# skhu101/TDNN-F_NAS

Measured on AMD Instinct MI355X. Metric: LF-MMI training frames/sec per node (SWBD 7q TDNN-F), higher is better.
Workload: dtype f32

## Files before the change

### include/tdnnf_hip.h

```cpp
#ifndef TDNNF_HIP_H_
#define TDNNF_HIP_H_

#include <stddef.h>
#include <stdint.h>

#ifdef __cplusplus
extern "C" {
#endif

#define TDNNF_OK 0
#define TDNNF_EINVAL 1
#define TDNNF_EHIP 2

#define TDNNF_MAX_OFFSETS 16

typedef struct {
  float *data;
  int rows, cols, stride;
} tdnnf_mat;

typedef void *tdnnf_stream;
typedef struct tdnnf_ng tdnnf_ng;

const char *tdnnf_last_error(void);
// ... 67 lines not shown
int tdnnf_batchnorm_compute_derived(const double *stats_dev, int D, float epsilon, float target_rms,
                                    float *scale_dev, float *offset_dev, tdnnf_stream stream);
int tdnnf_batchnorm_test_propagate(const tdnnf_mat *in, const float *scale_dev, const float *offset_dev,
                                   tdnnf_mat *out, tdnnf_stream stream);
int tdnnf_batchnorm_test_backprop(const tdnnf_mat *out_deriv, const float *scale_dev, tdnnf_mat *in_deriv,
                                  tdnnf_stream stream);


int tdnnf_softmax_flops_propagate(const tdnnf_mat *in, const float *gumbel_u_dev, float temp_proportion,
                                  tdnnf_mat *out, tdnnf_stream stream);
int tdnnf_softmax_flops_backprop(const tdnnf_mat *out_value, tdnnf_mat *out_deriv, float scale,
                                 const float *flops_dev, int dim, float temp_proportion,
                                 tdnnf_mat *in_deriv, tdnnf_stream stream);
int tdnnf_onehot_propagate(const float *sample_u_dev, tdnnf_mat *out, tdnnf_stream stream);
int tdnnf_onehot_backprop(const tdnnf_mat *out_deriv, float lr, float *output_acc_dev, void *workspace_dev,
                          size_t workspace_bytes, tdnnf_stream stream);
int tdnnf_copyn_propagate(const tdnnf_mat *in, float scale, tdnnf_mat *out, tdnnf_stream stream);
int tdnnf_copyn_backprop(const tdnnf_mat *out_deriv, float scale, tdnnf_mat *in_deriv, tdnnf_stream stream);
int tdnnf_constant_function_propagate(const float *output_dev, tdnnf_mat *out, tdnnf_stream stream);
int tdnnf_constant_function_backprop(const tdnnf_mat *out_deriv, float lr, float *output_acc_dev,
                                     void *workspace_dev, size_t workspace_bytes, tdnnf_stream stream);
int tdnnf_flops_constraint_backprop(const float *flops_dev, float scale, int rows_in, int cols_in,
                                    tdnnf_mat *in_deriv, tdnnf_stream stream);

int tdnnf_elementwise_product_propagate(const tdnnf_mat *in, int output_dim, tdnnf_mat *out, tdnnf_stream);
int tdnnf_elementwise_product_backprop(const tdnnf_mat *in_value, const tdnnf_mat *out_deriv, int output_dim,
                                       tdnnf_mat *in_deriv, tdnnf_stream);
int tdnnf_relu_propagate(const tdnnf_mat *in, tdnnf_mat *out, tdnnf_stream);
int tdnnf_relu_backprop(const tdnnf_mat *out_value, const tdnnf_mat *out_deriv, tdnnf_mat *in_deriv, tdnnf_stream);
int tdnnf_relu_repair(const double *stats_dev, int dim, float self_repair_scale, float lower, float upper,
                      tdnnf_mat *in_deriv, tdnnf_stream);
int tdnnf_relu_store_stats(const tdnnf_mat *out_value, double *stats_dev, void *workspace_dev,
                           size_t workspace_bytes, tdnnf_stream);
int tdnnf_affine_propagate(const tdnnf_mat *in, const float *W_dev, int ldw, const float *bias_dev, int Do,
                           tdnnf_mat *out, tdnnf_stream);
int tdnnf_affine_backprop(const tdnnf_mat *out_deriv, const float *W_dev, int ldw, int Di, tdnnf_mat *in_deriv,
                          tdnnf_stream);
int tdnnf_affine_update_simple(const tdnnf_mat *in_value, const tdnnf_mat *out_deriv, float lr, float *W_acc_dev,
                               int ldw, float *bias_acc_dev, void *workspace_dev, size_t workspace_bytes,
                               tdnnf_stream);
size_t tdnnf_affine_update_natural_gradient_workspace_bytes(int Do, int Di, int num_rows, int has_bias);
int tdnnf_affine_update_natural_gradient(const tdnnf_mat *in_value, const tdnnf_mat *out_deriv,
                                         tdnnf_ng *preconditioner_in, tdnnf_ng *preconditioner_out,
                                         float learning_rate, float *W_acc_dev, int ldw, float *bias_acc_dev,
                                         void *workspace_dev, size_t workspace_bytes, tdnnf_stream);
int tdnnf_log_softmax_propagate(const tdnnf_mat *in, tdnnf_mat *out, tdnnf_stream);
int tdnnf_log_softmax_backprop(const tdnnf_mat *out_value, const tdnnf_mat *out_deriv, tdnnf_mat *in_deriv,
                               tdnnf_stream);
int tdnnf_sum_scaled(const tdnnf_mat *a, float sa, const tdnnf_mat *b, float sb, tdnnf_mat *out, tdnnf_stream);
int tdnnf_add_scaled(const tdnnf_mat *a, float s, tdnnf_mat *out, tdnnf_stream);
int tdnnf_general_dropout(const tdnnf_mat *in, const float *mask_dev, int num_seq, tdnnf_mat *out, tdnnf_stream);
int tdnnf_general_dropout_mask(const float *uniform_dev, long long n, float proportion, int continuous, float *mask_dev, tdnnf_stream);

typedef struct tdnnf_den_graph tdnnf_den_graph;
typedef struct tdnnf_supervision tdnnf_supervision;

int tdnnf_den_graph_create(int num_states, int num_arcs, int num_pdfs, const int *arc_src, const int *arc_dst,
                           const int *arc_pdf, const float *arc_prob, const float *initial_probs, int start_state,
                           tdnnf_den_graph **out);
void tdnnf_den_graph_destroy(tdnnf_den_graph *);
int tdnnf_supervision_create(int num_sequences, int frames_per_sequence, const int *seq_state_begin,
                             const int *seq_arc_begin, const int *state_time, const float *final_logprob,
                             const int *arc_src, const int *arc_dst, const int *arc_pdf, const float *arc_logprob,
                             float weight, tdnnf_supervision **out);
void tdnnf_supervision_destroy(tdnnf_supervision *);

int tdnnf_chain_set_denominator_mode(int mode);
int tdnnf_chain_den_mw_status(int *fallbacks, int *disabled, int reset);
size_t tdnnf_chain_workspace_bytes(const tdnnf_den_graph *, int num_sequences, int frames_per_sequence);
int tdnnf_chain_objf_and_deriv(const tdnnf_den_graph *, const tdnnf_supervision *, const tdnnf_mat *nnet_output,
                               const tdnnf_mat *xent_output , float leaky_hmm_coefficient,
                               float l2_regularize, float xent_regularize, double *results_dev,
                               tdnnf_mat *nnet_output_deriv, tdnnf_mat *xent_deriv, void *workspace_dev,
                               size_t workspace_bytes, tdnnf_stream);

int tdnnf_ng_create(int rank, int update_period, float num_samples_history, float alpha, tdnnf_ng **out);
void tdnnf_ng_destroy(tdnnf_ng *);
int tdnnf_ng_freeze(tdnnf_ng *, int freeze);
int tdnnf_ng_precondition(tdnnf_ng *, tdnnf_mat *X, float *scale_host, tdnnf_stream);
size_t tdnnf_ng_stats_pass_workspace_bytes(int rank, int Di, int num_taps, int N);
int tdnnf_ng_stats_pass(const tdnnf_tdnn_indexes *ix, const tdnnf_mat *X, int Di, const float *eff_dev, const float *WT_dev,
                        const float *W_dev, int ldw, const float *bias_dev, tdnnf_mat *H, double *sumsq_dev, int sumsq_cap, int form,
                        void *workspace_dev, size_t workspace_bytes, tdnnf_stream);
const float *tdnnf_ng_scale_dev(const tdnnf_ng *);

size_t tdnnf_constrain_orthonormal_workspace_bytes(int rows, int cols);
int tdnnf_constrain_orthonormal(float scale, float *M_dev, int rows, int cols, int ld, void *workspace_dev,
                                size_t workspace_bytes, tdnnf_stream);
int tdnnf_axpy(const float *x_dev, float a, float *y_dev, size_t n, tdnnf_stream);
int tdnnf_dot(const float *x_dev, const float *y_dev, size_t n, double *result_host, tdnnf_stream);
size_t tdnnf_max_change_workspace_bytes(int num_comp);
int tdnnf_update_with_max_change(float *params_dev, float *delta_dev, int num_comp, const long long *comp_begin_host,
                                 const float *max_change_host, float max_param_change, float max_change_scale,
                                 float scale, int zero_delta, void *workspace_dev, size_t workspace_bytes,
                                 float *info_dev, tdnnf_stream);

int tdnnf_splice_input(const tdnnf_mat *feats, const tdnnf_mat *ivectors, int num_seq, int num_splice,
                       tdnnf_mat *out, tdnnf_stream);
int tdnnf_reorder_rows(const tdnnf_mat *in, int num_seq, int rho, int to_rho, tdnnf_mat *out, tdnnf_stream);

#define TDNNF_NET_MAX_LAYERS 32
typedef struct {
  int feat_dim, ivector_dim, num_pdfs;
  int hidden_dim, prefinal_small_dim;
  int num_layers;
  int bottleneck_dim[TDNNF_NET_MAX_LAYERS];
  int time_stride[TDNNF_NET_MAX_LAYERS];
  float bypass_scale;
  int frames_per_chunk, num_sequences;
  int frame_subsampling;
  float leaky_hmm, xent_regularize, chain_l2_regularize;
  float l2_hidden, l2_output;
  float max_change_hidden, max_change_output, max_param_change;
  float relu_self_repair_scale;
  float batchnorm_stats_scale;
  int darts_num_offsets;
  int darts_flags;
  float darts_temp_proportion;
  int use_natural_gradient;
  int bn_num_choices;
  int bn_choice_dims[8];
  int bn_mode;
  float bn_flops_scale;
  float bn_temp_proportion;
  int cv_update;
  int gemm_precision;
  int use_layer_offsets;
  int offset_left[TDNNF_NET_MAX_LAYERS];
  int offset_right[TDNNF_NET_MAX_LAYERS];
  int use_dropout;
} tdnnf_net_config;
typedef struct tdnnf_net tdnnf_net;

typedef struct tdnnf_egs_reader tdnnf_egs_reader;
typedef struct tdnnf_egs_writer tdnnf_egs_writer;
typedef struct tdnnf_eg tdnnf_eg;
int tdnnf_egs_reader_open(const char *path, tdnnf_egs_reader **out);
void tdnnf_egs_reader_close(tdnnf_egs_reader *);
int tdnnf_egs_reader_next(tdnnf_egs_reader *, tdnnf_eg **out);
void tdnnf_eg_destroy(tdnnf_eg *);
const char *tdnnf_eg_key(const tdnnf_eg *);
int tdnnf_eg_input_info(const tdnnf_eg *, const char *name, int *rows, int *cols, int *first_t);
int tdnnf_eg_input_copy(const tdnnf_eg *, const char *name, float *out);
int tdnnf_eg_supervision_info(const tdnnf_eg *, float *weight, int *num_sequences, int *frames_per_seq, int *label_dim, int *num_states,
                              int *num_arcs, int *first_t, int *t_step);
int tdnnf_egs_merge_sizes(const tdnnf_eg *const *egs, int n, int *num_states, int *num_arcs, int *frames_per_seq, int *feat_dim, int *ivector_dim);
int tdnnf_egs_merge(const tdnnf_eg *const *egs, int n, int first_t, int num_t, int frame_shift, float *feats, float *ivectors, int *seq_state_begin,
                    int *seq_arc_begin, int *state_time, float *final_logprob, int *arc_src, int *arc_dst, int *arc_pdf, float *arc_logprob,
                    float *weight_out);
int tdnnf_egs_writer_open(const char *path, tdnnf_egs_writer **out);
int tdnnf_egs_writer_close(tdnnf_egs_writer *);
int tdnnf_egs_writer_write(tdnnf_egs_writer *, const char *key, const float *feats, int rows, int feat_dim, int first_t, const float *ivector,
                           int ivector_dim, int compress, float weight, int frames, int t_step, int label_dim, int num_states, int num_arcs,
                           const float *final_logprob, const int *arc_src, const int *arc_dst, const int *arc_pdf, const float *arc_logprob);

int tdnnf_net_create(const tdnnf_net_config *cfg, tdnnf_net **out);
int tdnnf_net_create_shared(const tdnnf_net_config *cfg, const tdnnf_net *primary, tdnnf_net **out);
void tdnnf_net_destroy(tdnnf_net *);
long long tdnnf_net_num_params(const tdnnf_net *);
int tdnnf_net_num_components(const tdnnf_net *);
int tdnnf_net_component_info(const tdnnf_net *, int index, char *name_out, long long *begin, int *rows, int *cols,
                             int *has_bias, float *lr_factor, float *l2, float *max_change, float *orthonormal);
int tdnnf_net_component_num_alpha(const tdnnf_net *, int index);
int tdnnf_net_num_random_draws(const tdnnf_net *);
int tdnnf_net_set_random_draws(tdnnf_net *, const float *draws_dev);
int tdnnf_net_input_frames(const tdnnf_net *, int *num_t_in, int *first_t);
// ... 67 lines not shown
```

### tdnn-f_nas_amd/csrc/abi_tdnn.hip

```cpp
#include <dlfcn.h>
#include <stdlib.h>
#include <string.h>

#include <string>

#include "common.h"
#include "gemm_f32.h"
#include "planes_gemm.h"

namespace tdnnf {

static thread_local std::string g_last_error;

void set_error(const char *fmt, ...) {
  char buf[1024];
  va_list ap;
  va_start(ap, fmt);
  vsnprintf(buf, sizeof(buf), fmt, ap);
  va_end(ap);
  g_last_error = buf;
}
int hip_status(hipError_t e, const char *what) {
  set_error("HIP error %d (%s) in %s", (int)e, hipGetErrorString(e), what);
  return TDNNF_EHIP;
}

Options &options() {
  static Options o;
  return o;
}

namespace {
typedef int (*roctx_push_t)(const char *);
typedef int (*roctx_pop_t)();
roctx_push_t g_roctx_push = nullptr;
roctx_pop_t g_roctx_pop = nullptr;
bool roctx_ready() {
  static const bool ok = [] {
    const char *e = getenv("TDNNF_ROCTX");
    if (e && atoi(e) == 0) return false;
    for (const char *lib : {"librocprofiler-sdk-roctx.so", "librocprofiler-sdk-roctx.so.1", "libroctx64.so", "libroctx64.so.4"}) {
      void *h = dlopen(lib, RTLD_NOW | RTLD_GLOBAL);
      if (!h) continue;
      g_roctx_push = (roctx_push_t)dlsym(h, "roctxRangePushA");
      g_roctx_pop = (roctx_pop_t)dlsym(h, "roctxRangePop");
      if (g_roctx_push && g_roctx_pop) return true;
    }
    return false;
  }();
  return ok;
}
}
TraceRange::TraceRange(const char *name) : on(roctx_ready()) {
  if (on) g_roctx_push(name);
}
TraceRange::~TraceRange() {
  if (on) g_roctx_pop();
}

static bool tdnn_rows_ok(const tdnnf_tdnn_indexes *ix, int rows_in, int N) {
  if (!ix || ix->num_offsets < 1 || ix->num_offsets > TDNNF_MAX_OFFSETS || ix->row_stride < 1) return false;
  for (int i = 0; i < ix->num_offsets; i++) {
    const long long need = (long long)ix->row_offsets[i] + (long long)ix->row_stride * N - (ix->row_stride - 1);
    if (ix->row_offsets[i] < 0 || (N > 0 && rows_in < need)) return false;
  }
  return true;
}

}

using namespace tdnnf;

extern "C" {

const char *tdnnf_last_error(void) { return g_last_error.c_str(); }
int tdnnf_abi_version(void) { return 1; }

static int *option_slot(const char *name) {
  Options &o = options();
  if (!name) return nullptr;
  const struct { const char *n; int *p; } table[] = {{"ng_grouped", &o.ng_grouped}, {"ng_fuse", &o.ng_fuse}, {"ng_early_in", &o.ng_early_in},
                                                     {"wgrad_stream", &o.wgrad_stream}, {"gemm_ring", &o.gemm_ring}, {"planes", &o.planes}, {"den_split", &o.den_split}, {"phase_events", &o.phase_events}, {"wgrad_lag", &o.wgrad_lag}, {"ng_bk", &o.ng_bk}, {"ng_valu", &o.ng_valu}, {"ng_pform", &o.ng_pform}, {"planes_group", &o.planes_group}, {"xent_behind_den", &o.xent_behind_den}, {"ng_early_fork", &o.ng_early_fork}, {"ng_diag_skip", &o.ng_diag_skip}, {"wgrad_small", &o.wgrad_small}, {"splitk_per_cu", &o.splitk_per_cu}, {"gemm_alt_taps", &o.gemm_alt_taps}, {"reverse_passes", &o.reverse_passes}, {"splitk_partial_round", &o.splitk_partial_round}, {"wgrad_on_caller", &o.wgrad_on_caller}, {"den_mw_test_abort", &o.den_mw_test_abort}, {"planes_check_bound", &o.planes_check_bound}, {"den_gamma_pairs", &o.den_gamma_pairs}};
  for (auto &e : table)
    if (strcmp(e.n, name) == 0) return e.p;
  return nullptr;
}
int tdnnf_set_option(const char *name, int value) {
  int *p = option_slot(name);
  TDNNF_REQUIRE(p, "set_option: unknown option '%s' (ng_grouped, ng_fuse, ng_early_in, wgrad_stream, gemm_ring, planes, den_split)", name ? name : "(null)");
  *p = value;
  return TDNNF_OK;
}
int tdnnf_get_option(const char *name, int *value) {
  int *p = option_slot(name);
  TDNNF_REQUIRE(p && value, "get_option: unknown option '%s'", name ? name : "(null)");
  *value = *p;
  return TDNNF_OK;
}

}

namespace tdnnf {
int tdnn_propagate_impl(const tdnnf_tdnn_indexes *ix, const tdnnf_mat *in, const float *W, int ldw, int Do, int Di,
                        const float *bias, const float *eff_coef, int init_mode, int relu, tdnnf_mat *out, tdnnf_stream stream,
                        float *colstats, int *colstats_rows) {
  TDNNF_REQUIRE(mat_ok(in) && mat_ok(out) && W, "tdnn_propagate: bad matrices");
  TDNNF_REQUIRE(Do > 0 && Di > 0 && in->cols == Di && out->cols == Do, "tdnn_propagate: dims: in.cols=%d Di=%d out.cols=%d Do=%d",
                in ? in->cols : -1, Di, out ? out->cols : -1, Do);
  TDNNF_REQUIRE(tdnn_rows_ok(ix, in->rows, out->rows), "tdnn_propagate: input has too few rows for the time offsets");
  TDNNF_REQUIRE(ldw >= ix->num_offsets * Di, "tdnn_propagate: ldw < K*Di");
  TDNNF_REQUIRE(init_mode >= 0 && init_mode <= 2 && (init_mode != 1 || bias), "tdnn_propagate: init_mode 1 needs a bias");
  RowsGemmArgs a;
  memset(&a, 0, sizeof(a));
  a.A = in->data;
  a.lda = (long long)in->stride * ix->row_stride;
  a.B = W;
  a.ldb = ldw;
  a.C = out->data;
  a.ldc = out->stride;
  a.M = out->rows;
  a.N = Do;
  a.bias = bias;
  a.coef = eff_coef;
  a.init_mode = init_mode;
  a.relu = relu;
  a.colstats = colstats;
  a.colstats_rows = colstats_rows;
  a.nseg = ix->num_offsets;
  for (int i = 0; i < a.nseg; i++) {
    a.seg[i].a_off = (long long)ix->row_offsets[i] * in->stride;
    a.seg[i].b_off = (long long)i * Di;
    a.seg[i].klen = Di;
    a.seg[i].m_lo = 0;
    a.seg[i].m_hi = out->rows;
  }
  TDNNF_HIP(rows_gemm(a, true, (hipStream_t)stream));
  return TDNNF_OK;
}
}

extern "C" {

int tdnnf_tdnn_propagate(const tdnnf_tdnn_indexes *ix, const tdnnf_mat *in, const float *W, int ldw, int Do, int Di,
                         const float *bias, const float *eff_coef, int init_mode, tdnnf_mat *out, tdnnf_stream stream) {
  return tdnn_propagate_impl(ix, in, W, ldw, Do, Di, bias, eff_coef, init_mode, 0, out, stream);
}

}

namespace tdnnf {
int tdnn_backprop_data_impl(const tdnnf_tdnn_indexes *ix, const tdnnf_mat *out_deriv, const float *W, int ldw, int Do,
                            int Di, const float *eff_coef, int overwrite, const tdnnf_mat *add, float add_scale, int add_lo,
                            tdnnf_mat *in_deriv, tdnnf_stream stream) {
  TDNNF_REQUIRE(mat_ok(in_deriv) && mat_ok(out_deriv) && W, "tdnn_backprop_data: bad matrices");
  TDNNF_REQUIRE(Do > 0 && Di > 0 && in_deriv->cols == Di && out_deriv->cols == Do, "tdnn_backprop_data: bad dims");
  TDNNF_REQUIRE(tdnn_rows_ok(ix, in_deriv->rows, out_deriv->rows), "tdnn_backprop_data: in_deriv has too few rows for the time offsets");
  TDNNF_REQUIRE(ldw >= ix->num_offsets * Di, "tdnn_backprop_data: ldw < K*Di");
  const int rho = ix->row_stride, N = out_deriv->rows, K = ix->num_offsets;
  if (N == 0) return TDNNF_OK;
  for (int cls = 0; cls < rho; cls++) {
    RowsGemmArgs a;
    memset(&a, 0, sizeof(a));
    float cf_dummy = 0;
    (void)cf_dummy;
    int nseg = 0, u_max = 0;
// ... 171 lines not shown
```

### tdnn-f_nas_amd/csrc/common.h

```cpp
#pragma once
#include <hip/hip_runtime.h>
#include <stdarg.h>
#include <stdio.h>

#include "tdnnf_hip.h"

namespace tdnnf {

struct MatView {
  float *data;
  int rows, cols, stride;
};
inline MatView view(const tdnnf_mat *m) { return MatView{m->data, m->rows, m->cols, m->stride}; }

void set_error(const char *fmt, ...);
int hip_status(hipError_t e, const char *what);

inline bool mat_ok(const tdnnf_mat *m) {
  return m && m->rows >= 0 && m->cols >= 0 && m->stride >= m->cols && (m->data || m->rows * m->cols == 0);
}
inline bool same_dim(const tdnnf_mat *a, const tdnnf_mat *b) { return a->rows == b->rows && a->cols == b->cols; }

inline bool vec4_ok(const MatView &m) {
  return (reinterpret_cast<uintptr_t>(m.data) & 15) == 0 && m.stride % 4 == 0 && m.cols % 4 == 0;
}

#define TDNNF_REQUIRE(cond, ...)            \
  do {                                      \
    if (!(cond)) {                          \
      ::tdnnf::set_error(__VA_ARGS__);      \
      return TDNNF_EINVAL;                  \
    }                                       \
  } while (0)

#define TDNNF_HIP(expr)                                         \
  do {                                                          \
    hipError_t e__ = (expr);                                    \
    if (e__ != hipSuccess) return ::tdnnf::hip_status(e__, #expr); \
  } while (0)

#define TDNNF_LAUNCH_CHECK(name) TDNNF_HIP(hipGetLastError())

struct Options {
  int ng_grouped = 1;
  int ng_fuse = 1;
  int ng_early_in = 1;
  int wgrad_stream = -1;
  int gemm_ring = 1;
  int planes = 1;
  int den_mw_test_abort = 0;
  int planes_group = 1;
  int planes_check_bound = 0;
  int wgrad_lag = 3;
  int wgrad_on_caller = 0;
  int splitk_partial_round = 1;
  int reverse_passes = 0;
  int gemm_alt_taps = 1;
  int splitk_per_cu = 2;
  int wgrad_small = 0;
  int ng_bk = 0;
  int ng_early_fork = 1;
  int xent_behind_den = -1;
  int ng_pform = 1;
  int ng_valu = 0;
  int ng_diag_skip = 0;
  int phase_events = 0;
  int den_split = -1;
  int den_gamma_pairs = 0;
};
Options &options();

struct TraceRange {
  explicit TraceRange(const char *name);
  ~TraceRange();
  bool on;
};

__host__ __device__ inline float floor_keep_nan(float x, float f) { return x < f ? f : x; }

inline int grid_for(long long work, int block, int cap = 2048) {
  long long g = (work + block - 1) / block;
  if (g > cap) g = cap;
  if (g < 1) g = 1;
  return (int)g;
}

inline unsigned long long tdnnf_decision(unsigned long long step, unsigned long long k) {
  unsigned long long z = step * 0x9E3779B97F4A7C15ULL + k * 0xBF58476D1CE4E5B9ULL + 0x94D049BB133111EBULL;
  z = (z ^ (z >> 30)) * 0xBF58476D1CE4E5B9ULL;
  z = (z ^ (z >> 27)) * 0x94D049BB133111EBULL;
  return (z ^ (z >> 31)) >> 8;
}

constexpr int kFinCols = 8, kFinLanes = 32, kFinThreads = kFinCols * kFinLanes;
inline unsigned finalize_grid(int D) { return (unsigned)((D + kFinCols - 1) / kFinCols); }
#ifdef __HIPCC__
template <int NQ, class Acc>
__device__ __forceinline__ void finalize_sums(const float *partial, int chunks, long long qstride_rows, int D, int nq, Acc (&q)[NQ], Acc *red) {
  const int tc = threadIdx.x & (kFinCols - 1), lane = threadIdx.x / kFinCols, d = blockIdx.x * kFinCols + tc;
#pragma unroll
  for (int k = 0; k < NQ; k++) q[k] = 0;
  if (d < D) {
    const float *p = partial + d;
    const long long qs = qstride_rows * D;
    int c = lane;
    for (; c + 3 * kFinLanes < chunks; c += 4 * kFinLanes) {
      float v[NQ][4];
#pragma unroll
      for (int k = 0; k < NQ; k++) {
        if (k < nq) {
          const float *pk = p + (long long)k * qs;
          v[k][0] = pk[(long long)c * D]; v[k][1] = pk[(long long)(c + kFinLanes) * D];
          v[k][2] = pk[(long long)(c + 2 * kFinLanes) * D]; v[k][3] = pk[(long long)(c + 3 * kFinLanes) * D];
        }
      }
#pragma unroll
      for (int k = 0; k < NQ; k++) {
        if (k < nq) { q[k] += v[k][0]; q[k] += v[k][1]; q[k] += v[k][2]; q[k] += v[k][3]; }
      }
    }
    for (; c < chunks; c += kFinLanes) {
      float v[NQ];
#pragma unroll
      for (int k = 0; k < NQ; k++)
        if (k < nq) v[k] = p[(long long)k * qs + (long long)c * D];
#pragma unroll
      for (int k = 0; k < NQ; k++)
        if (k < nq) q[k] += v[k];
    }
  }
#pragma unroll
  for (int k = 0; k < NQ; k++) red[(k * kFinLanes + lane) * (kFinCols + 1) + tc] = q[k];
  __syncthreads();
  if (lane == 0) {
#pragma unroll
    for (int k = 0; k < NQ; k++) {
      Acc s = 0;
      for (int l = 0; l < kFinLanes; l++) s += red[(k * kFinLanes + l) * (kFinCols + 1) + tc];
      q[k] = s;
    }
  }
}
#endif

struct BnSync {
  int (*fn)(void *ctx, double *buf, long long count, tdnnf_stream stream);
  void *ctx;
  double *buf;
  int world;
};
BnSync *bn_sync_current();
// ... 52 lines not shown
```

### tdnn-f_nas_amd/csrc/fused.h

```cpp
#pragma once
#include "common.h"

namespace tdnnf {

struct PlanesSink {
  void *P;
  long long R;
  const float *rec;
};
hipError_t bn_apply_bypass(MatView x, const float *memo, int D, int period, MatView prev, float bypass, MatView out, hipStream_t s,
                           const float *mask = nullptr, int B = 1, const PlanesSink *planes = nullptr);

struct BwdPlanes {
  void *P;
  long long R;
  int lead;
  float *rec;
};

struct NgFuse {
  const float *W;
  int Rp, ldw;
  float *H;
  double *part;
  int part_cap;
};
bool bn_relu_bwd_ng_ok(MatView x, MatView dz, MatView d_aff, int Rp);
bool bn_relu_bwd_ng_pays(int rows);

size_t bn_relu_bwd_workspace_bytes(int rows, int cols);
hipError_t bn_relu_bwd(MatView x, MatView dz, float *memo, float target_rms, bool bn_test_mode, double *relu_stats, bool store_relu_stats,
                       bool self_repair, float self_repair_scale, MatView d_aff, float *bias_acc, float bias_scale,
                       void *ws, size_t ws_bytes, hipStream_t s, const float *mask = nullptr, int B = 1,
                       const NgFuse *ng = nullptr,
                       double *oderiv_stats = nullptr,
                       const BwdPlanes *planes = nullptr);

}
```

### tdnn-f_nas_amd/csrc/fused.hip

```cpp
#include <algorithm>

#include "common.h"
#include "fused.h"
#include "gemm_f32.h"
#include "planes_gemm.h"

namespace tdnnf {
namespace {

__device__ __forceinline__ void ld(const float *p, float (&v)[4], bool vec) {
  if (vec) {
    const float4 t = *reinterpret_cast<const float4 *>(p);
    v[0] = t.x; v[1] = t.y; v[2] = t.z; v[3] = t.w;
  } else {
    v[0] = p[0];
  }
}
__device__ __forceinline__ void st(float *p, const float (&v)[4], bool vec) {
  if (vec) *reinterpret_cast<float4 *>(p) = make_float4(v[0], v[1], v[2], v[3]);
  else p[0] = v[0];
}

__device__ __forceinline__ void store_planes4(const PlanesSink &pk, float ps, long long ra, int c, const float (&v)[4]) {
  typedef _Float16 h4 __attribute__((ext_vector_type(4)));
  h4 hi, lo;
#pragma unroll
  for (int j = 0; j < 4; j++) {
    const float w = v[j] * ps;
    hi[j] = (_Float16)w;
    lo[j] = (_Float16)(w - (float)hi[j]);
  }
  const int kb = c >> 4, k = c & 15, half = (k >> 3) ^ (int)((ra >> 3) & 1);
  _Float16 *dst = reinterpret_cast<_Float16 *>(pk.P) + (((long long)kb * 2) * pk.R + ra) * 16 + half * 8 + (k & 7);
  *reinterpret_cast<h4 *>(dst) = hi;
  *reinterpret_cast<h4 *>(dst + pk.R * 16) = lo;
}

template <int VEC, bool PLANES>
__global__ __launch_bounds__(256) void bn_apply_bypass_kernel(MatView x, const float *mean, const float *scale, int D, int period,
                                                              MatView prev, float bypass, MatView out, const float *mask, int B, PlanesSink pk, int rev) {
  const int cv = x.cols / VEC;
  const float ps = PLANES ? pk.rec[0] : 1.0f;
  const int ncb = PLANES ? cv / 8 : 1;
  const long long total = PLANES ? (long long)((x.rows + 7) / 8) * 8 * cv : (long long)x.rows * cv;
  for (long long e0 = blockIdx.x * 256LL + threadIdx.x; e0 < total; e0 += gridDim.x * 256LL) {
    const long long e = rev ? total - 1 - e0 : e0;
    int r, c;
    if (PLANES) {
      const long long blk = e >> 6;
      r = (int)(blk / ncb) * 8 + (int)((e >> 3) & 7);
      c = ((int)(blk % ncb) * 8 + (int)(e & 7)) * VEC;
      if (r >= x.rows) continue;
    } else {
      r = (int)(e / cv);
      c = (int)(e % cv) * VEC;
    }
    const int cd = c % period;
    if (cd >= D) continue;
    float xv[4], pv[4] = {0, 0, 0, 0}, o[4];
    ld(x.data + (long long)r * x.stride + c, xv, VEC == 4);
    if (prev.data) ld(prev.data + (long long)r * prev.stride + c, pv, VEC == 4);
    const float *mk = mask ? mask + (long long)(x.cols > D ? c / period : r % B) * D + cd : nullptr;
    float mu[4], sc[4], mv[4] = {1.f, 1.f, 1.f, 1.f};
    ld(mean + cd, mu, VEC == 4);
    ld(scale + cd, sc, VEC == 4);
    if (mk) ld(mk, mv, VEC == 4);
#pragma unroll
    for (int j = 0; j < VEC; j++) o[j] = (xv[j] - mu[j]) * sc[j] * mv[j] + bypass * pv[j];
    st(out.data + (long long)r * out.stride + c, o, VEC == 4);
    if constexpr (PLANES && VEC == 4) store_planes4(pk, ps, r, c, o);
  }
}

template <int VEC, bool RELU_STATS>
__global__ __launch_bounds__(256) void bn_relu_bwd_reduce_kernel(MatView x, MatView dz, const float *mean, const float *scale,
                                                                 int rows_per_chunk, int chunks, float *partial, const float *mask, int B) {
  __shared__ float red[5][4][64 * 4 + 4];
  const int tc = threadIdx.x & 63, tr = threadIdx.x >> 6;
  const int col = (blockIdx.x * 64 + tc) * VEC;
  const int r0 = blockIdx.y * rows_per_chunk, r1 = min(x.rows, r0 + rows_per_chunk);
  float s[5][4] = {};
  if (col < x.cols) {
    float mu[4], sc[4];
#pragma unroll
    for (int j = 0; j < VEC; j++) {
      mu[j] = mean[col + j];
      sc[j] = scale[col + j];
    }
    for (int r = r0 + tr; r < r1; r += 4) {
      float xv[4], dv[4];
      ld(x.data + (long long)r * x.stride + col, xv, VEC == 4);
      ld(dz.data + (long long)r * dz.stride + col, dv, VEC == 4);
      if (mask) {
        const float *mk = mask + (long long)(r % B) * x.cols + col;
#pragma unroll
        for (int j = 0; j < VEC; j++) dv[j] *= mk[j];
      }
#pragma unroll
      for (int j = 0; j < VEC; j++) {
        const float z = (xv[j] - mu[j]) * sc[j];
        s[0][j] += z * dv[j];
        s[1][j] += dv[j];
        s[2][j] += dv[j] * dv[j];
        if (RELU_STATS) {
          s[3][j] += xv[j];
          s[4][j] += xv[j] > 0.f ? 1.f : 0.f;
        }
      }
    }
  }
  constexpr int NQ = RELU_STATS ? 5 : 3;
#pragma unroll
  for (int q = 0; q < NQ; q++)
#pragma unroll
    for (int j = 0; j < VEC; j++) red[q][tr][tc * VEC + j] = s[q][j];
  __syncthreads();
  if (tr == 0 && col < x.cols) {
#pragma unroll
    for (int q = 0; q < NQ; q++)
#pragma unroll
      for (int j = 0; j < VEC; j++) {
        const int k = tc * VEC + j;
        partial[((long long)q * chunks + blockIdx.y) * x.cols + col + j] = (red[q][0][k] + red[q][1][k]) + (red[q][2][k] + red[q][3][k]);
      }
  }
}

__global__ __launch_bounds__(kFinThreads) void bn_relu_bwd_finalize_kernel(const float *partial, int chunks, int D, int N, float target_rms,
                                                                           float *memo, double *relu_stats, int test_mode, double *oderiv,
                                                                           double *sums_out = nullptr, const double *sums_in = nullptr, int N_local = 0,
                                                                           double *fro2 = nullptr, float repair_abs = 0.f) {
  __shared__ double red[5 * kFinLanes * (kFinCols + 1)];
  const int d = blockIdx.x * kFinCols + (threadIdx.x & (kFinCols - 1));
  double q[5];
  const int nq = relu_stats ? 5 : 3;
  if (!sums_in) finalize_sums<5, double>(partial, chunks, chunks, D, nq, q, red);
  if (sums_out) {
    if (threadIdx.x < kFinCols && d < D)
      for (int k = 0; k < nq; k++) sums_out[(size_t)k * D + d] = q[k];
    return;
  }
  if (relu_stats && blockIdx.x == 0 && threadIdx.x == 0) relu_stats[0] += (double)(sums_in ? N_local : N);
  if (oderiv && blockIdx.x == 0 && threadIdx.x == 0) oderiv[0] += (double)N;
  double bound = 0;
  if (threadIdx.x < kFinCols && d < D) {
    if (sums_in)
      for (int k = 0; k < nq; k++) q[k] = sums_in[(size_t)k * D + d];
    const float coeff = -1.0f / (target_rms * target_rms * N);
    const float sc = memo[2 * D + d];
    const float vdm = test_mode ? 0.f : (float)(coeff * q[0]) * sc;
    memo[3 * D + d] = vdm;
    memo[4 * D + d] = test_mode ? 0.f : (float)(-q[1] / N);
    if (relu_stats) {
      relu_stats[1 + d] += q[3];
      relu_stats[1 + D + d] += q[4];
    }
// ... 186 lines not shown
      }
      *reinterpret_cast<float4 *>(As + (rr + 32 * i) * LD + c4 * 4) = make_float4(o[i][0], o[i][1], o[i][2], o[i][3]);
    }
#pragma unroll
    for (int j = 0; j < NT; j++) {
      const int idx = t + 256 * j, n = idx >> 3, kk = (idx & 7) * 4;
      *reinterpret_cast<float4 *>(Bs + n * LD + kk) = wv[j];
    }
    if (k0 + BK < D) request(k0 + BK);
#pragma unroll
    for (int i = 0; i < 4; i++) {
      const int r = r0 + rr + 32 * i;
      if (FULL || r < x.rows) {
        st(d_aff.data + (long long)r * d_aff.stride + col, o[i], true);
        if constexpr (PLANES) store_planes4(pk, pks, (long long)pk_lead + r, col, o[i]);
      }
    }
#pragma unroll
    for (int j = 0; j < 4; j++) {
      float v = cs[j];
      v += __shfl_xor(v, 8, 64);
      v += __shfl_xor(v, 16, 64);
      v += __shfl_xor(v, 32, 64);
      if (lane < 8) colred[wave][lane * 4 + j] = v;
    }
    __syncthreads();
    {
      const float *as = As + (wave * 32 + li) * LD + lh * 4;
      const float *bs = Bs + li * LD + lh * 4;
#pragma unroll
      for (int kg = 0; kg < BK / 8; kg++) {
        const float4 a = *reinterpret_cast<const float4 *>(as + kg * 8);
#pragma unroll
        for (int j = 0; j < NT; j++) {
          const float4 b = *reinterpret_cast<const float4 *>(bs + j * 32 * LD + kg * 8);
          acc[j] = __builtin_amdgcn_mfma_f32_32x32x2f32(a.x, b.x, acc[j], 0, 0, 0);
          acc[j] = __builtin_amdgcn_mfma_f32_32x32x2f32(a.y, b.y, acc[j], 0, 0, 0);
          acc[j] = __builtin_amdgcn_mfma_f32_32x32x2f32(a.z, b.z, acc[j], 0, 0, 0);
          acc[j] = __builtin_amdgcn_mfma_f32_32x32x2f32(a.w, b.w, acc[j], 0, 0, 0);
        }
      }
    }
    if (t < BK) partial[(long long)blk * D + k0 + t] = (colred[0][t] + colred[1][t]) + (colred[2][t] + colred[3][t]);
    __syncthreads();
  }
#pragma unroll
  for (int j = 0; j < NT; j++) {
    const int n = j * 32 + li;
#pragma unroll
    for (int e = 0; e < 16; e++) {
      const int r = r0 + wave * 32 + (e & 3) + 8 * (e >> 2) + 4 * lh;
      if (n < ng.Rp && r < x.rows) ng.H[(long long)r * ng.Rp + n] = acc[j][e];
    }
  }
  double v = ssq;
  for (int o = 32; o > 0; o >>= 1) v += __shfl_xor(v, o, 64);
  if (lane == 0) red[wave] = v;
  __syncthreads();
  if (t == 0) ng.part[blk] = (red[0] + red[1]) + (red[2] + red[3]);
  if (blk == 0)
    for (int i = gridDim.x + t; i < ng.part_cap; i += 256) ng.part[i] = 0.0;
}

template <int NT, bool MASK, bool PLANES>
__global__ __launch_bounds__(256) void bn_relu_bwd_apply_ng_kernel(MatView x, MatView dz, const float *memo, int D, const double *repair_stats,
                                                                   float self_repair_scale, MatView d_aff, float *partial, const float *mask, int B,
                                                                   NgFuse ng, PlanesSink pk, int pk_lead, int rev) {
  const int blk = rev ? (int)gridDim.x - 1 - (int)blockIdx.x : (int)blockIdx.x;
  if (blk * 128 + 128 <= x.rows)
    bn_relu_bwd_apply_ng_body<NT, MASK, true, PLANES>(x, dz, memo, D, repair_stats, self_repair_scale, d_aff, partial, mask, B, ng, pk, pk_lead, blk);
  else bn_relu_bwd_apply_ng_body<NT, MASK, false, PLANES>(x, dz, memo, D, repair_stats, self_repair_scale, d_aff, partial, mask, B, ng, pk, pk_lead, blk);
}

__global__ __launch_bounds__(kFinThreads) void colsum_add_kernel(const float *partial, int chunks, int D, float scale, float *acc) {
  __shared__ float red[kFinLanes * (kFinCols + 1)];
  const int d = blockIdx.x * kFinCols + (threadIdx.x & (kFinCols - 1));
  float q[1];
  finalize_sums<1, float>(partial, chunks, chunks, D, 1, q, red);
  if (threadIdx.x < kFinCols && d < D) acc[d] += scale * q[0];
}

}

hipError_t bn_apply_bypass(MatView x, const float *memo, int D, int period, MatView prev, float bypass, MatView out, hipStream_t s, const float *mask, int B,
                           const PlanesSink *planes) {
  if (x.rows == 0) return hipSuccess;
  const bool vec = vec4_ok(x) && vec4_ok(out) && (!prev.data || vec4_ok(prev)) && D % 4 == 0 && (reinterpret_cast<uintptr_t>(memo) & 15) == 0 &&
                   (!mask || (reinterpret_cast<uintptr_t>(mask) & 15) == 0);
  const long long work = (long long)x.rows * (vec ? x.cols / 4 : x.cols);
  if (planes && !(vec && x.cols == D && D % 32 == 0 && planes->P && planes->rec)) return hipErrorInvalidValue;
  ProfHbmRange prof(4, 4.0 * x.rows * x.cols * ((prev.data ? 3.0 : 2.0) + (planes ? 1.0 : 0.0)), s);
  const PlanesSink none{nullptr, 0, nullptr};
  if (planes) hipLaunchKernelGGL((bn_apply_bypass_kernel<4, true>), dim3(grid_for((long long)((x.rows + 7) / 8) * 8 * (x.cols / 4), 256)), dim3(256), 0, s, x, memo, memo + 2 * D, D, period, prev, bypass, out, mask, B, *planes, 0);
  else if (vec) hipLaunchKernelGGL((bn_apply_bypass_kernel<4, false>), dim3(grid_for(work, 256)), dim3(256), 0, s, x, memo, memo + 2 * D, D, period, prev, bypass, out, mask, B, none, options().reverse_passes & 1);
  else hipLaunchKernelGGL((bn_apply_bypass_kernel<1, false>), dim3(grid_for(work, 256)), dim3(256), 0, s, x, memo, memo + 2 * D, D, period, prev, bypass, out, mask, B, none, 0);
  return hipGetLastError();
}

bool bn_relu_bwd_ng_ok(MatView x, MatView dz, MatView d_aff, int Rp) {
  return vec4_ok(x) && vec4_ok(dz) && vec4_ok(d_aff) && x.cols % 32 == 0 && Rp >= 1 && Rp <= 96 && x.rows >= 1;
}

bool bn_relu_bwd_ng_pays(int rows) {
  static int slots = 0;
  if (!slots) {
    int dev = 0, cus = 256;
    hipDeviceProp_t prop;
    if (hipGetDevice(&dev) == hipSuccess && hipGetDeviceProperties(&prop, dev) == hipSuccess) cus = prop.multiProcessorCount;
    slots = 2 * cus;
  }
  const int blocks = (rows + 127) / 128, rounds = (blocks + slots - 1) / slots;
  return 4 * blocks >= 3 * rounds * slots;
}

size_t bn_relu_bwd_workspace_bytes(int rows, int cols) {
  ColReducePlan p = colreduce_plan(rows, cols);
  const size_t blocks128 = ((size_t)rows + 127) / 128;
  return sizeof(float) * (5 * (size_t)p.chunks + std::max((size_t)p.chunks, blocks128)) * cols + 64;
}

hipError_t bn_relu_bwd(MatView x, MatView dz, float *memo, float target_rms, bool bn_test_mode, double *relu_stats, bool store_relu_stats,
                       bool self_repair, float self_repair_scale, MatView d_aff, float *bias_acc, float bias_scale,
                       void *ws, size_t ws_bytes, hipStream_t s, const float *mask, int B, const NgFuse *ng, double *oderiv_stats, const BwdPlanes *planes) {
  if (x.rows == 0) return hipSuccess;
  if (ws_bytes < bn_relu_bwd_workspace_bytes(x.rows, x.cols)) return hipErrorInvalidValue;
  if (ng && (!bn_relu_bwd_ng_ok(x, dz, d_aff, ng->Rp) || (reinterpret_cast<uintptr_t>(memo) & 15) || (reinterpret_cast<uintptr_t>(ng->W) & 15) || ng->ldw % 4))
    return hipErrorInvalidValue;
  const int D = x.cols;
  ProfHbmRange prof(5, 4.0 * x.rows * x.cols * 5.0, s);
  ColReducePlan pl = colreduce_plan(x.rows, D);
  const bool vec = vec4_ok(x) && vec4_ok(dz) && vec4_ok(d_aff);
  const int per = vec ? 256 : 64;
  dim3 grid((D + per - 1) / per, pl.chunks), block(256);
  float *partial = (float *)ws;
  float *bias_partial = partial + 5 * (size_t)pl.chunks * D;
  if (store_relu_stats) {
    if (vec) hipLaunchKernelGGL((bn_relu_bwd_reduce_kernel<4, true>), grid, block, 0, s, x, dz, memo, memo + 2 * D, pl.rows_per_chunk, pl.chunks, partial, mask, B);
    else hipLaunchKernelGGL((bn_relu_bwd_reduce_kernel<1, true>), grid, block, 0, s, x, dz, memo, memo + 2 * D, pl.rows_per_chunk, pl.chunks, partial, mask, B);
  } else {
    if (vec) hipLaunchKernelGGL((bn_relu_bwd_reduce_kernel<4, false>), grid, block, 0, s, x, dz, memo, memo + 2 * D, pl.rows_per_chunk, pl.chunks, partial, mask, B);
    else hipLaunchKernelGGL((bn_relu_bwd_reduce_kernel<1, false>), grid, block, 0, s, x, dz, memo, memo + 2 * D, pl.rows_per_chunk, pl.chunks, partial, mask, B);
  }
  double *fro2 = fro_bound_buf();
  if (fro2 && fro_bound_blocks()) *fro_bound_blocks() = (int)finalize_grid(D);
  const float repair_abs = self_repair ? 2.0f * fabsf(self_repair_scale) : 0.f;
  if (BnSync *sy = bn_test_mode ? nullptr : bn_sync_current()) {
    hipLaunchKernelGGL(bn_relu_bwd_finalize_kernel, dim3(finalize_grid(D)), dim3(kFinThreads), 0, s, partial, pl.chunks, D, x.rows, target_rms, memo,
                       store_relu_stats ? relu_stats : (double *)nullptr, 0, (double *)nullptr, sy->buf, (const double *)nullptr, 0);
    if (sy->fn(sy->ctx, sy->buf, 3LL * D, (tdnnf_stream)s)) return hipErrorUnknown;
    hipLaunchKernelGGL(bn_relu_bwd_finalize_kernel, dim3(finalize_grid(D)), dim3(kFinThreads), 0, s, partial, pl.chunks, D, x.rows * sy->world, target_rms, memo,
                       store_relu_stats ? relu_stats : (double *)nullptr, 0, oderiv_stats, (double *)nullptr, (const double *)sy->buf, x.rows, fro2, repair_abs);
  } else {
    hipLaunchKernelGGL(bn_relu_bwd_finalize_kernel, dim3(finalize_grid(D)), dim3(kFinThreads), 0, s, partial, pl.chunks, D, x.rows, target_rms, memo,
                       store_relu_stats ? relu_stats : (double *)nullptr, bn_test_mode ? 1 : 0, oderiv_stats, (double *)nullptr, (const double *)nullptr, 0, fro2,
                       repair_abs);
  }
  const double *rep = self_repair ? relu_stats : nullptr;
  PlanesSink pk{nullptr, 0, nullptr};
  int pk_lead = 0;
  if (planes && planes->P) {
    if (!(fro2 && vec && x.cols % 16 == 0)) return hipErrorInvalidValue;
    hipError_t e = planes_scale_bound(fro2, (int)finalize_grid(D), (double)x.rows * D, 1.0f, 0.0f, nullptr, planes->rec, s);
    if (e != hipSuccess) return e;
    pk = PlanesSink{planes->P, planes->R, planes->rec};
    pk_lead = planes->lead;
  }
  if (ng) {
    const int blocks = (x.rows + 127) / 128;
#define APPLY_NG(NT)                                                                                                                                     \
// ... 22 lines not shown
```

### tdnn-f_nas_amd/csrc/net.h

```cpp
#pragma once
#include <hip/hip_runtime.h>

#include <string>
#include <utility>
#include <vector>

#include <map>

#include "common.h"
#include "planes_gemm.h"
#include "tdnnf_hip.h"

namespace tdnnf {
struct RowsGemmGroup;
struct PlanesSplitGroup;

struct NgGroup;
struct NgFin;
struct UpdGroup;

struct Grid {
  int t0, step, n;
  int last() const { return t0 + step * (n - 1); }
};
// ... 5 lines not shown
  float lr_factor, l2, max_change, orthonormal;
  int num_alpha;
  bool plain = false;
  bool updatable = true;
  long long size() const { return (long long)rows * cols + num_alpha + (has_bias ? rows : 0); }
};

struct Tdnn {
  int comp;
  int Di, Do, K;
  int offsets[TDNNF_MAX_OFFSETS];
  Grid in, out;
  bool darts;
  int share, draw0;
  float *memo;
  int *active;
  tdnnf_tdnn_indexes ix;
  int rows_in, rows_out;
};

struct TdnnfLayer {
  int stride, bn;
  int left, right;
  Tdnn lin, aff;
  Grid gin, gout, glin;
  bool perm;
  int bypass_row0, bypass_rowstep;
  float *lin_out, *lin_perm, *relu_out, *noop_out;
  float *bn_memo;
  double *bn_stats, *relu_stats;
  int c_arch, arch_draw0;
  float *arch_p, *arch_mask, *lin_masked;
};

}

struct tdnnf_net {
  tdnnf_net_config cfg;
  std::vector<tdnnf::CompDesc> comps;
  long long num_params;
  float *params, *grads;
  float *paramsT;
  int planes_np = 0;
  struct PlaneSlot {
    void *P = nullptr, *PT = nullptr;
    size_t bytesP = 0, bytesPT = 0;
    float *scale = nullptr;
    long long last[5] = {-1, -1, -1, -1, -1};
  };
  std::map<const float *, PlaneSlot> plane_slots;
  std::vector<tdnnf::PlanesOperand> pw;
  std::vector<float *> pw_scale;
  void *planes_ws = nullptr;
  double *fro_buf = nullptr;
  int B, T, Tout;
  tdnnf::Grid g_lda, g_feat;
  tdnnf::Tdnn tdnn1;
  std::vector<tdnnf::TdnnfLayer> layers;
  int c_lda, c_prefinal_l;
  struct Head {
    int c_affine, c_linear, c_output;
    float *aff_relu, *bn1_out, *lin_out, *bn2_out, *y;
    float *bn1_memo, *bn2_memo;
    double *bn1_stats, *bn2_stats, *relu_stats;
  } head[2];
  float *xent_logsoftmax;
  char *arena;
  size_t arena_bytes;
  float *lda_in, *lda_out, *t1_relu, *t1_bn;
  float *t1_bn_memo;
  double *t1_bn_stats, *t1_relu_stats;
  float *prefinal_l_out;
  float *dA, *dB, *dC, *d_small, *d_small2;
  float *d_y, *d_xent;
  float *tapgrad;
  double *tapdots;
  const float *draws;
  std::vector<tdnnf_ng *> ng_in, ng_out;
  float *orthoT;
  struct NgComp {
    float *H_in = nullptr, *H_out = nullptr, *T = nullptr, *bsum = nullptr;
    double *part_in = nullptr, *part_out = nullptr;
    int N = 0;
  };
  std::vector<NgComp> ngc;
  float *ng_bsum_all = nullptr;
  size_t ng_bsum_floats = 0;
  float *ngTmp = nullptr;
  void *ng_side_ws = nullptr;
  size_t ngset_ws_bytes = 0;
  struct NgBucket {
    int key;
    std::vector<int> comps;
    tdnnf::NgGroup *group;
  };
  std::vector<NgBucket> ng_buckets;
  std::vector<int> ng_cur;
  tdnnf::NgFin *ngfin = nullptr;
  bool ng_grouped = true;
  hipEvent_t ev_ngc = nullptr;
  hipStream_t s3;
  hipEvent_t ev_s3;
  hipEvent_t ev_fin0, ev_fin;
  float *s3_scratch;
  size_t s3_scratch_bytes;
  bool wg_on;
  hipStream_t s4;
  hipEvent_t ev_pg[4], ev_pg_in;
  int wg_lag = 3;
  float *dC2 = nullptr, *dS[2] = {nullptr, nullptr};
  unsigned pg_count;
  void *ws4;
  void *ws2;
  float *s2_scratch;
  float *s4_scratch;
  hipStream_t s5 = nullptr;
  void *ws5 = nullptr;
  float *s5_scratch = nullptr;
  struct EarlyIn {
    unsigned char xin[256];
    long long recorded = -1, done = -1;
  };
  std::vector<EarlyIn> early;
  long long fb_count = 0;
  bool early_on = false, early_any = false;
  bool early_group = false;
  tdnnf::RowsGemmGroup *early_launch = nullptr;
  tdnnf::PlanesSplitGroup *wsplit_group = nullptr;
  hipEvent_t ev_early_in = nullptr, ev_early = nullptr;
  size_t s4_scratch_bytes;
  bool wg_two;
  float *gtmp;
  std::vector<char> oderiv_nonzero_own;
  std::vector<char> *oderiv_nonzero = &oderiv_nonzero_own;
  tdnnf::BnSync bn_sync{nullptr, nullptr, nullptr, 1};
  enum { kPhases = 8 };
  hipEvent_t ev_phase[kPhases] = {nullptr, nullptr, nullptr, nullptr, nullptr, nullptr, nullptr, nullptr};
  bool phase_rec[kPhases] = {false, false, false, false, false, false, false, false};
  tdnnf::UpdGroup *upd = nullptr;
  bool den_split = true;
  hipStream_t s2;
  hipEvent_t ev_fork, ev_den, ev_num;
  hipEvent_t ev_den_rec = nullptr;
  hipEvent_t ev_comm = nullptr;
  int num_draws;
  bool owns_ng = true;
  int dropout_draw0;
  float *dropout_masks;
  float dropout_proportion;
  void *ws;
  size_t ws_bytes;
  void *chain_ws;
  size_t chain_ws_bytes;
  std::vector<std::pair<std::string, tdnnf_mat>> named;
  struct GradBucket {
    long long begin, end;
    int close_key;
    hipEvent_t ready, handoff;
  };
  std::vector<GradBucket> buckets;
  bool capture_on = false;
  std::vector<float *> captured;
};

namespace tdnnf {
int net_layer_grids(const tdnnf_net_config &c, int Tout, std::vector<TdnnfLayer> &layers, Grid *g_lda);
void net_make_tdnn(Tdnn *t, int comp, int Di, int Do, const std::vector<int> &offs, const Grid &in, const Grid &out, int B);
inline float *net_W(const tdnnf_net *n, int comp) { return n->params + n->comps[comp].begin; }
inline float *net_alpha(const tdnnf_net *n, int comp) {
  const CompDesc &c = n->comps[comp];
  return c.num_alpha ? n->params + c.begin + (long long)c.rows * c.cols : nullptr;
}
inline float *net_bias(const tdnnf_net *n, int comp) {
  const CompDesc &c = n->comps[comp];
  return c.has_bias ? n->params + c.begin + (long long)c.rows * c.cols + c.num_alpha : nullptr;
}
}
```

### tdnn-f_nas_amd/csrc/net.hip

```cpp
#include <math.h>
#include <string.h>

#include <functional>
#include <string>
#include <vector>

#include "common.h"
#include "fused.h"
#include "gemm_f32.h"
#include "gemm_ring.h"
#include "net.h"
#include "ng.h"
#include "optim_group.h"

namespace tdnnf {
namespace {

struct UpdTable {
  long long begin[129];
  float lr[128];
  float l2coef[128];
};

__global__ void add_scaled_taps_kernel(const float *G, const float *coef, float *acc, int Do, int KDi, int Di) {
// ... 316 lines not shown
  const bool lag3 = wg_size && n->wg_lag == 3;
  n->dC2 = lag3 ? A.mat(max_rows, Hd) : nullptr;
  n->dS[0] = lag3 ? A.mat(std::max(max_lin_rows, No), std::max(S, 512)) : nullptr;
  n->dS[1] = lag3 ? A.mat(std::max(max_lin_rows, No), std::max(S, 512)) : nullptr;
  size_t tg = 0;
  for (auto &L : n->layers)
    if (L.lin.darts) tg = std::max(tg, (size_t)L.bn * L.lin.K * Hd);
  n->tapgrad = tg ? A.take<float>(tg) : nullptr;
  n->tapdots = A.take<double>(TDNNF_TAP_DOTS_DOUBLES(TDNNF_MAX_OFFSETS));
  n->bn_sync.buf = A.take<double>(5 * (size_t)std::max(std::max(Hd, S), 1) + 8);
  n->dropout_masks = (c.use_dropout && !c.cv_update) ? A.take<float>((size_t)(c.num_layers + 1) * B * Hd) : nullptr;
  n->gtmp = A.take<float>((size_t)n->num_params + 16);
  n->paramsT = (n->cfg.gemm_precision == 1 || n->cfg.gemm_precision == 2) ? A.take<float>((size_t)n->num_params + 16) : nullptr;
  n->planes_np = n->cfg.gemm_precision == 3 ? 2 : (n->cfg.gemm_precision == 2 && options().planes ? 3 : 0);
  n->plane_slots.clear();
  n->pw.assign(n->comps.size(), PlanesOperand());
  n->pw_scale.assign(n->comps.size(), nullptr);
  n->planes_ws = nullptr;
  n->fro_buf = nullptr;
  if (n->planes_np) {
    const int np = n->planes_np;
    int lead_cap = 0;
    for (auto &L : n->layers)
      for (const Tdnn *td : {&L.lin, &L.aff})
        for (int i = 0; i < td->K; i++) lead_cap = std::max(lead_cap, td->ix.row_offsets[i]);
    auto slot = [&](const float *key, int rows, int cols, bool with_lead) {
      const long long R = planes_rows_padded((long long)(with_lead ? 2 * ((lead_cap + 15) & ~15) : 0) + rows + 256);
      const long long Rt = planes_rows_padded(((cols + 255) / 256) * 256LL);
      tdnnf_net::PlaneSlot ps;
      ps.bytesP = planes_bytes(np, R, (planes_kblocks(cols) + 15) / 16 * 16);
      ps.bytesPT = planes_bytes(np, Rt, planes_t_kblocks(rows));
      ps.P = A.take<char>(ps.bytesP + 64);
      ps.PT = A.take<char>(ps.bytesPT + 64);
      ps.scale = A.take<float>(4);
      if (A.base) n->plane_slots[key] = ps;
    };
    const int big_rows = std::max(max_rows, std::max(N0, No)), small_rows = std::max(max_lin_rows, No), small_cols = std::max(S, 512);
    slot(n->lda_out, N0, lda_dim, false);
    slot(n->t1_bn, N0, Hd, false);
    for (auto &L : n->layers) {
      slot(L.noop_out, N_of(L.gout, B), Hd, false);
      slot(L.lin_out, N_of(L.lin.out, B), L.bn, false);
      if (L.c_arch >= 0) slot(L.lin_masked, N_of(L.lin.out, B), L.bn, false);
    }
    slot(n->prefinal_l_out, No, S, false);
    for (int h = 0; h < 2; h++) {
      slot(n->head[h].bn1_out, No, Hd, false);
      slot(n->head[h].bn2_out, No, S, false);
    }
    slot(n->d_y, No, P, false);
    slot(n->d_xent, No, P, false);
    slot(n->dA, big_rows, Hd, true);
    slot(n->dB, big_rows, Hd, true);
    slot(n->dC, big_rows, Hd, true);
    slot(n->d_small, small_rows, small_cols, true);
    slot(n->d_small2, small_rows, small_cols, true);
    n->planes_ws = A.take<char>(planes_sumsq_ws_bytes() + 64);
    n->fro_buf = A.take<double>(finalize_grid(std::max(Hd, S)) + 8);
    for (size_t i = 0; i < n->comps.size(); i++) {
      const CompDesc &cd = n->comps[i];
      if (cd.plain || cd.rows < 2 || (int)i == n->c_lda) continue;
      PlanesOperand &o = n->pw[i];
      o.rows = cd.rows; o.cols = cd.cols; o.ld = cd.cols; o.np = np; o.lead = 0;
      o.R = planes_rows_padded(((cd.rows + 255) / 256) * 256LL);
      o.Rt = planes_rows_padded(((cd.cols + 255) / 256) * 256LL);
      o.P = A.take<char>(planes_bytes(np, o.R, planes_kblocks(cd.cols)) + 64);
      o.PT = A.take<char>(planes_bytes(np, o.Rt, planes_t_kblocks(cd.rows)) + 64);
      n->pw_scale[i] = A.take<float>(4);
      o.scale = n->pw_scale[i];
    }
  }
  n->s3_scratch = nullptr;
  n->s3_scratch_bytes = 0;
  n->ng_grouped = options().ng_grouped != 0;
  size_t tall = 0, tall_ws = 0;
  for (auto &cd : n->comps)
    if (cd.orthonormal != 0.f && cd.rows > cd.cols) {
      tall = std::max(tall, (size_t)cd.rows * cd.cols);
      tall_ws = std::max(tall_ws, tdnnf_constrain_orthonormal_workspace_bytes(cd.cols, cd.rows));
    }
  n->orthoT = tall ? A.take<float>(tall + 16) : nullptr;
  size_t ng_ws = 0;
  n->ngc.assign(n->comps.size(), tdnnf_net::NgComp());
  if (n->cfg.use_natural_gradient) {
    size_t mtmp = 0;
    auto comp_ng = [&](int comp, int K, int rows) {
      const CompDesc &cd = n->comps[comp];
      if (!cd.updatable || cd.plain) return;
      const int Dx = cd.cols + (cd.has_bias ? 1 : 0), ldT = (Dx + 3) & ~3;
      const int rank_in = std::min(20, (Dx + 1) / 2), rank_out = std::min(80, (cd.rows + 1) / 2);
      const int Rpi = (rank_in + 3) & ~3, Rpo = (rank_out + 3) & ~3;
      mtmp = std::max(mtmp, std::max((size_t)cd.rows * Rpi, (size_t)Rpo * ldT));
      ng_ws = std::max(ng_ws, std::max(ng_stats_workspace_bytes(rank_in, Dx, K, rows), ng_stats_workspace_bytes(rank_out, cd.rows, 1, rows)));
      auto &S = n->ngc[comp];
      S.N = rows;
      S.H_in = A.take<float>((size_t)rows * Rpi + 64);
      S.H_out = A.take<float>((size_t)rows * Rpo + 64);
      S.T = A.take<float>((size_t)cd.rows * ldT + 16);
      S.bsum = nullptr;
      S.part_in = A.take<double>((size_t)rows_gemm_sumsq_blocks(rows) + 8);
      S.part_out = A.take<double>((size_t)rows_gemm_sumsq_blocks(rows) + 8);
    };
    const int No_ = n->Tout * B;
    comp_ng(n->tdnn1.comp, 1, N0);
    for (auto &L : n->layers) {
      comp_ng(L.lin.comp, L.lin.K, L.lin.rows_out);
      comp_ng(L.aff.comp, L.aff.K, L.aff.rows_out);
    }
    comp_ng(n->c_prefinal_l, 1, No_);
    for (int h = 0; h < 2; h++) {
      comp_ng(n->head[h].c_affine, 1, No_);
      comp_ng(n->head[h].c_linear, 1, No_);
      comp_ng(n->head[h].c_output, 1, No_);
    }
    {
      size_t tot = 0;
      for (size_t i = 0; i < n->comps.size(); i++)
        if (n->ngc[i].N > 0) tot += ((size_t)n->comps[i].rows + 15) & ~(size_t)15;
      n->ng_bsum_floats = tot;
      n->ng_bsum_all = A.take<float>(tot + 16);
      size_t o = 0;
      for (size_t i = 0; i < n->comps.size(); i++)
        if (n->ngc[i].N > 0) {
          n->ngc[i].bsum = n->ng_bsum_all ? n->ng_bsum_all + o : nullptr;
          o += ((size_t)n->comps[i].rows + 15) & ~(size_t)15;
        }
    }
    const size_t maxN = (size_t)std::max(std::max(max_rows, N0), No_);
    n->ngset_ws_bytes = wgrad_workspace_bytes(80, 80, 1, (int)maxN) + 256;
    n->ngTmp = A.take<float>(mtmp + 64);
    n->ng_side_ws = A.take<char>(n->ngset_ws_bytes);
    n->s3_scratch_bytes = 16u << 20;
    n->s3_scratch = A.take<float>(n->s3_scratch_bytes / sizeof(float));
  }
  size_t ws = 0;
  auto upd = [&](size_t b) { ws = std::max(ws, b); };
  upd(wgrad_workspace_bytes(Hd, lda_dim, 1, N0));
  upd(colreduce_bytes(max_rows, Hd));
  upd(sizeof(float) * 2 * (size_t)Hd * rows_gemm_colstats_cap(std::max(max_rows, std::max(N0, No))));
  upd(bn_relu_bwd_workspace_bytes(max_rows, Hd));
  for (auto &L : n->layers) {
    upd(wgrad_workspace_bytes(L.lin.Do, L.lin.Di, L.lin.K, L.lin.rows_out));
    upd(wgrad_workspace_bytes(L.aff.Do, L.aff.Di, L.aff.K, L.aff.rows_out));
    upd(tdnnf_constrain_orthonormal_workspace_bytes(L.bn, L.lin.K * Hd));
  }
  upd(wgrad_workspace_bytes(S, Hd, 1, No));
  upd(wgrad_workspace_bytes(Hd, S, 1, No));
  upd(wgrad_workspace_bytes(P, S, 1, No));
  upd(colreduce_bytes(No, P));
  upd(tdnnf_constrain_orthonormal_workspace_bytes(S, Hd));
  upd(tdnnf_max_change_workspace_bytes((int)n->comps.size()));
  upd(ng_ws);
  upd(tall_ws);
  if (n->cfg.bn_num_choices > 0) upd(sizeof(float) * (size_t)((max_lin_rows + 511) / 512 + 1) * 512);
  n->ws_bytes = ws + 256;
  n->ws = A.take<char>(n->ws_bytes);
  n->wg_on = options().wgrad_stream >= 0 ? options().wgrad_stream != 0 : std::max(max_rows, N0) <= 32768;
  n->early_on = n->cfg.use_natural_gradient && n->ng_grouped && (options().ng_early_in >= 2 || (options().ng_early_in != 0 && !n->wg_on));
  n->early_group = n->early_on && n->wg_on && options().ng_early_in == 3;
  const bool s4_used = n->wg_on || n->early_on;
  n->ws4 = s4_used ? A.take<char>(n->ws_bytes) : nullptr;
  n->s4_scratch_bytes = s4_used ? (32u << 20) : 0;
  n->s4_scratch = s4_used ? A.take<float>(n->s4_scratch_bytes / sizeof(float)) : nullptr;
  const bool two = n->wg_on && options().wgrad_stream != 1;
  n->ws2 = two ? A.take<char>(n->ws_bytes) : nullptr;
  n->s2_scratch = two ? A.take<float>(n->s4_scratch_bytes / sizeof(float)) : nullptr;
  const bool three = two && options().wgrad_stream == 3;
  n->ws5 = three ? A.take<char>(n->ws_bytes) : nullptr;
  n->s5_scratch = three ? A.take<float>(n->s4_scratch_bytes / sizeof(float)) : nullptr;
}

static int phase_mark(tdnnf_net *n, int k, hipStream_t s) {
  if (!tdnnf::options().phase_events) return TDNNF_OK;
  if (!n->ev_phase[k]) TDNNF_HIP(hipEventCreate(&n->ev_phase[k]));
  TDNNF_HIP(hipEventRecord(n->ev_phase[k], s));
  n->phase_rec[k] = true;
  return TDNNF_OK;
}

#define CK(expr)             \
  do {                       \
    int rc__ = (expr);       \
    if (rc__) return rc__;   \
  } while (0)
// ... 712 lines not shown
    auto it = n->plane_slots.find(m.data);
    if (it == n->plane_slots.end() || m.rows <= 0) return TDNNF_OK;
    tdnnf_net::PlaneSlot &ps = it->second;
    if (m.cols >= 1024) want = kP;
    PlanesSplitArgs a;
    a.np = np; a.x = view(&m); a.lead = lead; a.scale = ps.scale; a.sumsq_ws = n->planes_ws;
    if (np == 2 && fb.blocks > 0 && (fb.add_coef == 0.f || fb.add_rec)) {
      a.fro2_bound = n->fro_buf; a.fro2_blocks = fb.blocks; a.fro_mul = fb.mul; a.add_coef = fb.add_coef; a.add_rec = fb.add_rec;
    }
    lead = (lead + 15) & ~15;
    a.lead = lead;
    a.R = planes_rows_padded((long long)2 * lead + m.rows + 256);
    a.Rt = planes_rows_padded(((m.cols + 255) / 256) * 256LL);
    a.P = (want & kP) ? ps.P : nullptr;
    a.PT = (want & kT) ? ps.PT : nullptr;
    const long long kb_alloc = (planes_kblocks(m.cols) + 15) / 16 * 16;
    TDNNF_REQUIRE(planes_bytes(np, a.R, kb_alloc) <= ps.bytesP && planes_bytes(np, a.Rt, planes_t_kblocks(m.rows)) <= ps.bytesPT,
                  "net_forward_backward: plane slot too small for a %d x %d matrix", m.rows, m.cols);
    const long long cfg5[5] = {m.rows, m.cols, lead, a.R, want};
    a.pads_done = memcmp(cfg5, ps.last, sizeof(cfg5)) == 0;
    memcpy(ps.last, cfg5, sizeof(cfg5));
    TDNNF_HIP(planes_split(a, st));
    o->base = m.data; o->rows = m.rows; o->cols = m.cols; o->ld = m.stride; o->np = np;
    o->P = a.P; o->R = a.R; o->lead = lead; o->kb_alloc = kb_alloc; o->PT = a.PT; o->Rt = a.Rt; o->scale = np == 2 ? ps.scale : nullptr;
    return TDNNF_OK;
  };
  auto hint_of = [&](const PlanesOperand &o) -> const PlanesOperand * { return o.base ? &o : nullptr; };
  std::vector<PlanesSplitArgs> wsplits;
  bool darts_coef_done = false;
  auto split_weights = [&](int comp, const float *coef, int period, bool group = false) -> int {
    PlanesOperand &o = n->pw[comp];
    if (!o.P) return TDNNF_OK;
    o.base = Wp(n, comp);
    o.coef = coef;
    o.coef_period = period;
    PlanesSplitArgs a;
    a.np = np; a.x = MatView{Wp(n, comp), o.rows, o.cols, o.cols}; a.lead = 0; a.R = o.R; a.P = const_cast<void *>(o.P); a.Rt = o.Rt;
    a.PT = const_cast<void *>(o.PT); a.scale = n->pw_scale[comp]; a.sumsq_ws = n->planes_ws;
    a.col_coef = coef; a.col_coef_period = period;
    o.scale = np == 2 ? n->pw_scale[comp] : nullptr;
    a.pads_done = n->fb_count > 1;
    if (group && options().planes_group && planes_split_group_ok(a)) wsplits.push_back(a);
    else TDNNF_HIP(planes_split(a, s));
    return TDNNF_OK;
  };
  if (pl_on) {
    for (size_t i = 0; i < n->comps.size(); i++)
      if (n->comps[i].num_alpha == 0 || n->comps[i].plain) CK(split_weights((int)i, nullptr, 0, true));
    if (options().planes_group && n->draws) {
      for (auto &L : n->layers) {
        if (!L.lin.darts) continue;
        for (Tdnn *td : {&L.lin, &L.aff}) {
          const float *u = n->draws + td->draw0;
          CK(tdnnf_tdnn_darts_coef(Ap(n, td->comp), td->K, c.darts_flags, c.darts_temp_proportion, u, u + td->K, td->share, td->memo,
                                   td->memo + TDNNF_MAX_OFFSETS, s));
          hipLaunchKernelGGL(active_taps_kernel, dim3(1), dim3(64), 0, s, td->memo + TDNNF_MAX_OFFSETS, td->K, td->active);
        }
        CK(split_weights(L.lin.comp, L.lin.memo + TDNNF_MAX_OFFSETS, c.hidden_dim, true));
        CK(split_weights(L.aff.comp, L.aff.memo + TDNNF_MAX_OFFSETS, L.bn, true));
      }
      darts_coef_done = true;
    }
    TDNNF_HIP(planes_split_group(wsplits, &n->wsplit_group, s));
  }
  auto wplanes = [&](int comp) -> const PlanesOperand * { return pl_on && n->pw[comp].P ? &n->pw[comp] : nullptr; };
  auto bwd_planes = [&](const tdnnf_mat &d, int lead, BwdPlanes *bp, PlanesOperand *po) -> int {
    *bp = BwdPlanes{nullptr, 0, 0, nullptr};
    *po = PlanesOperand();
    if (!(pl_on && np == 2 && d.cols % 16 == 0 && d.cols >= 1024)) return TDNNF_OK;
    auto it = n->plane_slots.find(d.data);
    if (it == n->plane_slots.end()) return TDNNF_OK;
    tdnnf_net::PlaneSlot &ps = it->second;
    lead = (lead + 15) & ~15;
    const long long R = planes_rows_padded((long long)2 * lead + d.rows + 256), kb_alloc = (planes_kblocks(d.cols) + 15) / 16 * 16;
    TDNNF_REQUIRE(planes_bytes(np, R, kb_alloc) <= ps.bytesP, "net_forward_backward: plane slot too small for a %d x %d matrix", d.rows, d.cols);
    const long long cfg5[5] = {d.rows, d.cols, lead, R, kP};
    if (memcmp(cfg5, ps.last, sizeof(cfg5)) != 0) TDNNF_HIP(planes_pad(np, ps.P, planes_kblocks(d.cols), R, lead, d.rows, s));
    memcpy(ps.last, cfg5, sizeof(cfg5));
    *bp = BwdPlanes{ps.P, R, lead, ps.scale};
    po->base = d.data; po->rows = d.rows; po->cols = d.cols; po->ld = d.stride; po->np = np;
    po->P = ps.P; po->R = R; po->lead = lead; po->kb_alloc = kb_alloc; po->scale = ps.scale;
    return TDNNF_OK;
  };
  auto bn_apply_planes = [&](const tdnnf_mat &x, const float *memo, const MatView &byp, float bypass, const tdnnf_mat &out, const float *mask, const FroBound &fb,
                             PlanesOperand *po) -> int {
    *po = PlanesOperand();
    auto it = (pl_on && np == 2 && fb.blocks > 0 && (fb.add_coef == 0.f || fb.add_rec) && out.cols == Hd && out.stride == ldpad(Hd)) ? n->plane_slots.find(out.data)
                                                                                                                                         : n->plane_slots.end();
    if (it == n->plane_slots.end()) {
      TDNNF_HIP(bn_apply_bypass(view(&x), memo, Hd, ldpad(Hd), byp, bypass, view(&out), s, mask, B));
      return TDNNF_OK;
    }
    tdnnf_net::PlaneSlot &ps = it->second;
    const long long R = planes_rows_padded((long long)out.rows + 256), kb_alloc = (planes_kblocks(out.cols) + 15) / 16 * 16;
    TDNNF_REQUIRE(planes_bytes(np, R, kb_alloc) <= ps.bytesP, "net_forward_backward: plane slot too small for a %d x %d matrix", out.rows, out.cols);
    TDNNF_HIP(planes_scale_bound(n->fro_buf, fb.blocks, (double)out.rows * out.cols, fb.mul, fb.add_coef, fb.add_rec, ps.scale, s));
    const long long cfg5[5] = {out.rows, out.cols, 0, R, kP};
    if (memcmp(cfg5, ps.last, sizeof(cfg5)) != 0 && ps.last[0] >= 0) {
      TDNNF_HIP(planes_pad(np, ps.P, planes_kblocks(out.cols), R, 0, out.rows, s));
    }
    memcpy(ps.last, cfg5, sizeof(cfg5));
    const PlanesSink sink{ps.P, R, ps.scale};
    TDNNF_HIP(bn_apply_bypass(view(&x), memo, Hd, ldpad(Hd), byp, bypass, view(&out), s, mask, B, &sink));
    if (options().planes_check_bound) TDNNF_HIP(planes_check_bound(view(&out), ps.scale, n->planes_ws, s));
    po->base = out.data; po->rows = out.rows; po->cols = out.cols; po->ld = out.stride; po->np = np;
    po->P = ps.P; po->R = R; po->lead = 0; po->kb_alloc = kb_alloc; po->scale = ps.scale;
    return TDNNF_OK;
  };
  TransposedWeightsScope gemm_wt(n->params, n->paramsT, n->paramsT ? n->num_params : 0);
  if (n->paramsT) {
    TransTable tb;
    memset(&tb, 0, sizeof(tb));
    const int nc = (int)n->comps.size();
    for (int i = 0; i < nc; i++) {
      tb.begin[i] = n->comps[i].begin;
      tb.rows[i] = n->comps[i].rows;
      tb.cols[i] = n->comps[i].cols;
    }
    hipLaunchKernelGGL(transpose_weights_kernel, dim3(256, nc), dim3(256), 0, s, n->params, n->paramsT, tb);
  }
  TDNNF_REQUIRE(n->chain_ws_bytes >= tdnnf_chain_workspace_bytes(den, B, n->Tout) - (n->den_split ? 0 : chain_split_region_bytes(den, B, n->Tout)),
                "net_forward_backward: denominator graph changed size");
  unsigned long long coin_k = 0;
  auto coin = [&]() { return (int)(::tdnnf::tdnnf_decision((unsigned long long)step, 2 * coin_k++) & 1); };

  TraceRange trace_step("tdnnf_net_forward_backward");
  const int N0 = N_of(n->g_lda, B);
  tdnnf_mat lda_in = M(n->lda_in, N0, lda_dim), lda_out = M(n->lda_out, N0, lda_dim);
  CK(tdnnf_splice_input(feats, ivectors, B, 3, &lda_in, s));
  CK(tdnnf_affine_propagate(&lda_in, Wp(n, n->c_lda), lda_dim, Bp(n, n->c_lda), lda_dim, &lda_out, s));
  tdnnf_tdnn_indexes ix1;
  memset(&ix1, 0, sizeof(ix1));
  ix1.row_stride = 1;
  ix1.num_offsets = 1;
  tdnnf_mat t1r = M(n->t1_relu, N0, Hd), t1b = M(n->t1_bn, N0, Hd);
  const MatView none{nullptr, 0, 0, 0};
  const bool drop = n->dropout_masks && n->dropout_proportion > 0.f;
  if (drop) {
    TDNNF_REQUIRE(n->draws, "net_forward_backward: dropout needs net_set_random_draws before every step");
    const long long nm = (long long)(c.num_layers + 1) * B * Hd;
    hipLaunchKernelGGL(dropout_mask_kernel, dim3(grid_for(nm, 256)), dim3(256), 0, s, n->draws + n->dropout_draw0, n->dropout_proportion, nm, n->dropout_masks);
  }
  auto mask_of = [&](int m) -> const float * { return drop ? n->dropout_masks + (size_t)m * B * Hd : nullptr; };
  std::vector<PlanesOperand> po_in(n->layers.size()), po_lin(n->layers.size());
  PlanesOperand po_lda, po_top, po_pl, po_b1[2], po_b2[2];
  CK(split(lda_out, 0, kP | kT, &po_lda, s));
  FroBound fb_next;
  const float mask_max = drop ? 1.0f + 2.0f * n->dropout_proportion : 1.0f;
  {
    PlanesHintScope ph(hint_of(po_lda), wplanes(n->tdnn1.comp));
    FroBoundScope fbs(pl_on ? n->fro_buf : nullptr, &fb_next.blocks);
    CK(affine_relu_bn_stats(n, &ix1, &lda_out, Wp(n, n->tdnn1.comp), lda_dim, Hd, lda_dim, Bp(n, n->tdnn1.comp), nullptr, &t1r, n->t1_bn_memo, n->t1_bn_stats, s));
  }
  fb_next.mul = mask_max;
  PlanesOperand po_next;
  CK(bn_apply_planes(t1r, n->t1_bn_memo, none, 0.f, t1b, mask_of(0), fb_next, &po_next));
  float *prev = n->t1_bn;
  int layer_no = 0;
  for (auto &L : n->layers) {
    layer_no++;
    TraceRange trace_layer(("forward tdnnf" + std::to_string(layer_no + 1)).c_str());
    tdnnf_mat in = M(prev, N_of(L.gin, B), Hd);
    tdnnf_mat lin = M(L.lin_out, L.lin.rows_out, L.bn);
    const float *lin_eff = nullptr, *aff_eff = nullptr;
    if (L.lin.darts) {
      TDNNF_REQUIRE(n->draws, "net_forward_backward: a DARTS net needs net_set_random_draws before every step");
      if (!darts_coef_done)
        for (Tdnn *td : {&L.lin, &L.aff}) {
          const float *u = n->draws + td->draw0;
          CK(tdnnf_tdnn_darts_coef(Ap(n, td->comp), td->K, c.darts_flags, c.darts_temp_proportion, u, u + td->K, td->share, td->memo,
                                   td->memo + TDNNF_MAX_OFFSETS, s));
          hipLaunchKernelGGL(active_taps_kernel, dim3(1), dim3(64), 0, s, td->memo + TDNNF_MAX_OFFSETS, td->K, td->active);
        }
      lin_eff = L.lin.memo + TDNNF_MAX_OFFSETS;
      aff_eff = L.aff.memo + TDNNF_MAX_OFFSETS;
      if (pl_on && !darts_coef_done) {
        CK(split_weights(L.lin.comp, lin_eff, Hd));
        CK(split_weights(L.aff.comp, aff_eff, L.bn));
      }
    }
    ProfFlopsScale taps_active(L.lin.darts && (c.darts_flags & TDNNF_DARTS_UNIFORM_SAMPLE) && L.lin.K > 2 ? 2.0 / L.lin.K : 1.0);
    const bool use_pl = pl_on;
    if (use_pl) {
      if (po_next.base == in.data && po_next.rows == in.rows) po_in[layer_no - 1] = po_next;
      else CK(split(in, 0, kP | kT, &po_in[layer_no - 1], s, fb_next));
    }
    fb_next = FroBound();
    po_next = PlanesOperand();
    {
      PlanesHintScope ph(hint_of(po_in[layer_no - 1]), wplanes(L.lin.comp));
      CK(tdnnf_tdnn_propagate(&L.lin.ix, &in, Wp(n, L.lin.comp), L.lin.K * Hd, L.bn, Hd, nullptr, lin_eff, 2, &lin, s));
    }
    tdnnf_mat aff_in = lin;
    if (L.c_arch >= 0) {
      TDNNF_REQUIRE(n->draws || c.bn_mode == 1, "net_forward_backward: the bottleneck supernet needs net_set_random_draws before every step");
      hipLaunchKernelGGL(bn_choice_forward_kernel, dim3(1), dim3(256), 0, s, bn_choice(c), Wp(n, L.c_arch),
                         n->draws ? n->draws + L.arch_draw0 : nullptr, L.arch_p, L.arch_mask);
      aff_in = M(L.lin_masked, L.lin.rows_out, L.bn);
      hipLaunchKernelGGL(col_scale_kernel, dim3(grid_for((long long)lin.rows * L.bn, 256)), dim3(256), 0, s, view(&lin), L.arch_mask, view(&aff_in));
    }
    if (L.perm) {
      tdnnf_mat src = aff_in;
      aff_in = M(L.lin_perm, L.lin.rows_out, L.bn);
      CK(tdnnf_reorder_rows(&src, B, L.aff.ix.row_stride, 1, &aff_in, s));
    }
    tdnnf_mat relu = M(L.relu_out, L.aff.rows_out, Hd);
    if (use_pl && !L.perm) CK(split(aff_in, 0, kP | kT, &po_lin[layer_no - 1], s));
    {
      PlanesHintScope ph(hint_of(po_lin[layer_no - 1]), wplanes(L.aff.comp));
      FroBoundScope fbs(pl_on ? n->fro_buf : nullptr, &fb_next.blocks);
      CK(affine_relu_bn_stats(n, &L.aff.ix, &aff_in, Wp(n, L.aff.comp), L.aff.K * L.bn, Hd, L.bn, Bp(n, L.aff.comp), aff_eff, &relu, L.bn_memo, L.bn_stats, s));
    }
    fb_next.mul = mask_max;
    fb_next.add_coef = c.bypass_scale;
    fb_next.add_rec = po_in[layer_no - 1].base ? po_in[layer_no - 1].scale : nullptr;
    if (c.bypass_scale != 0.f && !fb_next.add_rec) fb_next.blocks = 0;
    tdnnf_mat byp = sub_grid_view(prev, L.gin, L.gout, B, Hd);
    tdnnf_mat x = relu, out = M(L.noop_out, L.aff.rows_out, Hd);
    if (byp.rows != out.rows) {
      x = tdnnf_mat{L.relu_out, L.gout.n, byp.cols, B * ldpad(Hd)};
      out = tdnnf_mat{L.noop_out, L.gout.n, byp.cols, B * ldpad(Hd)};
    }
    if (byp.rows == relu.rows) CK(bn_apply_planes(x, L.bn_memo, view(&byp), c.bypass_scale, out, mask_of(layer_no), fb_next, &po_next));
    else TDNNF_HIP(bn_apply_bypass(view(&x), L.bn_memo, Hd, ldpad(Hd), view(&byp), c.bypass_scale, view(&out), s, mask_of(layer_no), B));
    prev = L.noop_out;
  }
  CK(phase_mark(n, 1, s));
  const bool use_ng = c.use_natural_gradient != 0;
  auto finish_refreshes = [&]() -> int {
    if (use_ng && n->ng_grouped) {
      if (!n->ngfin) {
        bool ready = false;
        for (tdnnf_ng *g : all_ng()) ready = ready || ng_dim(g) != 0;
        if (ready) CK(ng_fin_create(all_ng(), &n->ngfin));
      }
      if (n->ngfin) {
        int did = 0;
        SplitKScratchOverride side_scratch(n->s3_scratch, n->s3_scratch_bytes);
        CK(ng_fin_run(n->ngfin, n->s3, true, &did));
        if (did) {
          TDNNF_HIP(hipEventRecord(n->ev_fin, n->s3));
          early_refresh = true;
        }
      }
    }
    if (early_refresh) TDNNF_HIP(hipStreamWaitEvent(s, n->ev_fin, 0));
    return TDNNF_OK;
  };
  n->early_any = false;
  auto is_head_comp = [&](int comp) { return comp == n->c_prefinal_l || comp == n->head[0].c_affine || comp == n->head[0].c_linear || comp == n->head[0].c_output ||
                                             comp == n->head[1].c_affine || comp == n->head[1].c_linear || comp == n->head[1].c_output; };
  auto launch_early_in = [&](int which) -> int {
    if (!(use_ng && n->early_on)) return TDNNF_OK;
    bool forked = false;
    if (n->early_group) {
      std::vector<RowsGemmArgs> calls;
      std::vector<int> who;
      for (int comp = (int)n->comps.size() - 1; comp >= 0; comp--) {
        auto &E = n->early[comp];
        if (E.done == n->fb_count || (which == 0 && is_head_comp(comp))) continue;
        if (E.recorded != n->fb_count - 1 || !n->ng_in[comp] || !n->ng_out[comp] || ng_dim(n->ng_in[comp]) == 0 || ng_dim(n->ng_out[comp]) == 0) continue;
        if (n->comps[comp].lr_factor == 0.f || !n->ngc[comp].H_in) continue;
        NgInput xin;
        memcpy(&xin, E.xin, sizeof(xin));
        if (!forked) {
          TDNNF_HIP(hipEventRecord(n->ev_early_in, s));
          TDNNF_HIP(hipStreamWaitEvent(n->s4, n->ev_early_in, 0));
          if (early_refresh) TDNNF_HIP(hipStreamWaitEvent(n->s4, n->ev_fin, 0));
          forked = true;
        }
        RowsGemmArgs a;
        CK(ng_stats_main_prepare(n->ng_in[comp], xin, n->ngc[comp].H_in, n->ngc[comp].part_in, n->s4, &a));
        if (!rows_gemm_group_ok(a)) continue;
        calls.push_back(a);
        who.push_back(comp);
      }
      if (!calls.empty()) {
        TDNNF_HIP(rows_gemm_group(calls, &n->early_launch, n->s4));
        for (int comp : who) n->early[comp].done = n->fb_count;
        TDNNF_HIP(hipEventRecord(n->ev_early, n->s4));
        n->early_any = true;
      }
      return TDNNF_OK;
    }
    SplitKScratchOverride early_scratch(n->s4_scratch, n->s4_scratch_bytes);
    for (int comp = (int)n->comps.size() - 1; comp >= 0; comp--) {
      auto &E = n->early[comp];
      if (E.done == n->fb_count || (which == 0 && is_head_comp(comp))) continue;
      if (E.recorded != n->fb_count - 1 || !n->ng_in[comp] || !n->ng_out[comp] || ng_dim(n->ng_in[comp]) == 0 || ng_dim(n->ng_out[comp]) == 0) continue;
      if (n->comps[comp].lr_factor == 0.f || !n->ngc[comp].H_in) continue;
      if (!forked) {
        TDNNF_HIP(hipEventRecord(n->ev_early_in, s));
        TDNNF_HIP(hipStreamWaitEvent(n->s4, n->ev_early_in, 0));
        if (early_refresh) TDNNF_HIP(hipStreamWaitEvent(n->s4, n->ev_fin, 0));
        forked = true;
      }
      NgInput xin;
      memcpy(&xin, E.xin, sizeof(xin));
      CK(ng_stats_main(n->ng_in[comp], xin, n->ngc[comp].H_in, n->ngc[comp].part_in, n->ws4, n->ws_bytes, n->s4));
      E.done = n->fb_count;
    }
    if (forked) {
      TDNNF_HIP(hipEventRecord(n->ev_early, n->s4));
      n->early_any = true;
    }
    return TDNNF_OK;
  };
  const bool early_at_fork = n->early_on && !n->wg_on && !n->early_group && options().ng_early_fork != 0;
  if (early_at_fork) {
    CK(finish_refreshes());
    CK(launch_early_in(0));
  }
  const int No = n->Tout * B;
  tdnnf_mat top = M(prev, No, Hd), pl = M(n->prefinal_l_out, No, S);
  if (po_next.base == top.data && po_next.rows == top.rows) po_top = po_next;
  else CK(split(top, 0, kP | kT, &po_top, s, fb_next));
  {
    PlanesHintScope ph(hint_of(po_top), wplanes(n->c_prefinal_l));
    CK(tdnnf_affine_propagate(&top, Wp(n, n->c_prefinal_l), Hd, nullptr, S, &pl, s));
  }
  CK(split(pl, 0, kP | kT, &po_pl, s));
  tdnnf_mat y = M(n->head[0].y, No, P), dy = M(n->d_y, No, P), dx = M(n->d_xent, No, P);
  tdnnf_mat lsm = M(n->xent_logsoftmax, No, P);
  for (int h = 0; h < 2; h++) {
    auto &H = n->head[h];
    tdnnf_mat ar = M(H.aff_relu, No, Hd), lo = M(H.lin_out, No, S), b1 = M(H.bn1_out, No, Hd), b2 = M(H.bn2_out, No, S), yh = M(H.y, No, P);
    FroBound fb_b1;
    {
      PlanesHintScope ph(hint_of(po_pl), wplanes(H.c_affine));
      FroBoundScope fbs(pl_on ? n->fro_buf : nullptr, &fb_b1.blocks);
      CK(affine_relu_bn_stats(n, &ix1, &pl, Wp(n, H.c_affine), S, Hd, S, Bp(n, H.c_affine), nullptr, &ar, H.bn1_memo, H.bn1_stats, s));
    }
    CK(bn_apply_planes(ar, H.bn1_memo, none, 0.f, b1, nullptr, fb_b1, &po_b1[h]));
    if (!po_b1[h].base) CK(split(b1, 0, kP | kT, &po_b1[h], s, fb_b1));
    {
      PlanesHintScope ph(hint_of(po_b1[h]), wplanes(H.c_linear));
      CK(tdnnf_affine_propagate(&b1, Wp(n, H.c_linear), Hd, nullptr, S, &lo, s));
    }
    CK(bn_fwd(n, H.lin_out, H.bn2_out, No, S, H.bn2_memo, H.bn2_stats, s));
    CK(split(b2, 0, kP | kT, &po_b2[h], s));
    {
      PlanesHintScope ph(hint_of(po_b2[h]), wplanes(H.c_output));
      CK(tdnnf_affine_propagate(&b2, Wp(n, H.c_output), S, Bp(n, H.c_output), P, &yh, s));
    }
    if (h == 0) {
      TraceRange trace_den("chain denominator forward-backward (second stream)");
      TDNNF_HIP(hipEventRecord(n->ev_fork, s));
      TDNNF_HIP(hipStreamWaitEvent(n->s2, n->ev_fork, 0));
      const bool den_split = n->den_split;
      TDNNF_HIP(hipStreamWaitEvent(n->s3, n->ev_fork, 0));
      const int xbd = options().xent_behind_den;
      const bool behind = den_split && (xbd > 0 || (xbd < 0 && !n->wg_on));
      if (behind && !n->ev_den_rec) TDNNF_HIP(hipEventCreateWithFlags(&n->ev_den_rec, hipEventDisableTiming));
      bool rec = false;
      CK(chain_den(den, sup, &y, c.leaky_hmm, &dy, n->chain_ws, n->s2, !den_split, n->s3, behind ? n->ev_den_rec : nullptr, &rec));
      if (rec) TDNNF_HIP(hipStreamWaitEvent(s, n->ev_den_rec, 0));
      TDNNF_HIP(hipEventRecord(n->ev_den, n->s2));
      hipStream_t sn = n->s3;
      if (n->wg_on && den_split) {
        sn = n->s4;
        TDNNF_HIP(hipStreamWaitEvent(sn, n->ev_fork, 0));
      }
      CK(chain_num_recursion(sup, den, &y, n->chain_ws, sn));
      TDNNF_HIP(hipEventRecord(n->ev_num, sn));
    }
  }
  tdnnf_mat yx = M(n->head[1].y, No, P);
  const bool dense_first = log_softmax_propagate_with_aux(&yx, &lsm, &dx, -c.xent_regularize * chain_supervision_weight(sup), s);
  if (!dense_first) CK(tdnnf_log_softmax_propagate(&yx, &lsm, s));
  TDNNF_HIP(hipStreamWaitEvent(s, n->ev_num, 0));
  CK(chain_num_xent(den, sup, &y, &lsm, c.xent_regularize, &dx, n->chain_ws, s, dense_first));
  if (!dense_first) CK(tdnnf_log_softmax_backprop(&lsm, &dx, &dx, s));

  CK(phase_mark(n, 2, s));
  auto capture = [&](const std::string &name, const tdnnf_mat &m) -> int {
    if (!n->capture_on) return TDNNF_OK;
    tdnnf_mat *dst = nullptr;
    for (auto &kv : n->named)
      if (kv.first == name) dst = &kv.second;
    if (!dst) {
      float *p = nullptr;
      TDNNF_HIP(hipMalloc((void **)&p, sizeof(float) * (size_t)std::max(1, m.rows) * ldpad(m.cols)));
// ... 57 lines not shown
      if (gb.close_key != key) continue;
      hipStream_t cs = s;
      if (!use_ng && n->wg_on && n->pg_count > 0) {
        for (unsigned b = 1; b <= side_streams() && b <= n->pg_count; b++) TDNNF_HIP(hipStreamWaitEvent(s, n->ev_pg[(n->pg_count - b) & 3], 0));
      }
      if (use_ng) {
        TDNNF_HIP(hipEventRecord(gb.handoff, s));
        TDNNF_HIP(hipStreamWaitEvent(n->s3, gb.handoff, 0));
        cs = n->s3;
      }
      const long long cnt = gb.end - gb.begin;
      if (cnt > 0)
        hipLaunchKernelGGL(commit_grads_kernel, dim3(grid_for(cnt, 256)), dim3(256), 0, cs, n->grads + gb.begin, n->gtmp + gb.begin, cnt, results);
      TDNNF_HIP(hipEventRecord(gb.ready, cs));
    }
    return TDNNF_OK;
  };
  auto bias_target = [&](int comp) -> float * {
    if (n->comps[comp].lr_factor == 0.f) return nullptr;
    if (!use_ng) return Bg(n, comp);
    return n->ngc[comp].bsum;
  };
  bool den_joined = false;
  bool caller_used = false;
  auto param_grad = [&](int comp, const tdnnf_tdnn_indexes &ix, int K, int Di, int Do, tdnnf_mat *x, tdnnf_mat *dyv, const float *eff,
                        bool bias_done, const int *active, int max_active, bool from_tapgrad) -> int {
    const int ldw = K * Di;
    float *bias_acc = Bg(n, comp);
    if (n->comps[comp].lr_factor == 0.f) return TDNNF_OK;
    hipStream_t sw = s;
    void *wsw = n->ws;
    const bool on_caller = n->wg_on && options().wgrad_on_caller != 0 && n->early_any && !den_joined;
    if (on_caller) caller_used = true;
    float *scr = nullptr;
    if (n->wg_on && !on_caller) {
      const int ns = (n->wg_two ? 2 : 1) + (n->s5 ? 1 : 0), k = (int)(n->pg_count % (unsigned)ns);
      const int which = k == 0 ? 0 : (k == 1 && n->wg_two) ? 1 : 2;
      sw = which == 0 ? n->s4 : which == 1 ? n->s2 : n->s5;
      wsw = which == 0 ? n->ws4 : which == 1 ? n->ws2 : n->ws5;
      scr = which == 0 ? n->s4_scratch : which == 1 ? n->s2_scratch : n->s5_scratch;
      TDNNF_HIP(hipEventRecord(n->ev_pg_in, s));
      TDNNF_HIP(hipStreamWaitEvent(sw, n->ev_pg_in, 0));
    }
    SplitKScratchOverride sw_scratch(scr, scr ? n->s4_scratch_bytes : 0);
    auto handed_off = [&]() -> int {
      if (!n->wg_on || on_caller) return TDNNF_OK;
      TDNNF_HIP(hipEventRecord(n->ev_pg[n->pg_count & 3], sw));
      const unsigned lag = lag3 ? 3u : 1u;
      if (n->pg_count >= lag) TDNNF_HIP(hipStreamWaitEvent(s, n->ev_pg[(n->pg_count - lag) & 3], 0));
      n->pg_count++;
      return TDNNF_OK;
    };
    if (!use_ng) {
      CK(tdnn_update_simple_impl(&ix, x, dyv, Do, Di, eff, 1.0f, Wg(n, comp), ldw, bias_done ? nullptr : bias_acc, wsw, n->ws_bytes, active, max_active, sw));
      return handed_off();
    }
    const int N = dyv->rows, ones = bias_acc ? 1 : 0, Dx = ldw + ones, ldT = (Dx + 3) & ~3;
    auto &S = n->ngc[comp];
    TDNNF_REQUIRE(S.T && S.N == N, "net_forward_backward: component %s has no natural-gradient buffers for %d rows", n->comps[comp].name.c_str(), N);
    float *T = S.T;
    const bool grouped = n->ng_grouped && ng_dim(n->ng_in[comp]) != 0 && ng_dim(n->ng_out[comp]) != 0;
    const bool overwrite = !from_tapgrad && !active && eff == nullptr && (ones || ldT == ldw);
    if (!overwrite) TDNNF_HIP(hipMemsetAsync(T, 0, sizeof(float) * (size_t)Do * ldT, sw));
    if (from_tapgrad)
      hipLaunchKernelGGL(scaled_taps_to_kernel, dim3(grid_for((long long)Do * ldw, 256)), dim3(256), 0, sw, n->tapgrad, eff, Do, ldw, Di, T, ldT);
    else
      CK(tdnn_update_simple_impl(&ix, x, dyv, Do, Di, eff, 1.0f, T, ldT, nullptr, wsw, n->ws_bytes, active, max_active, sw, overwrite));
    if (ones) {
      if (!bias_done) TDNNF_HIP(colsum_add(view(dyv), 1.0f, S.bsum, wsw, sw));
      if (!grouped) hipLaunchKernelGGL(set_column_kernel, dim3((Do + 255) / 256), dim3(256), 0, sw, S.bsum, Do, T, ldT, ldw);
    }
    NgInput xin;
    memset(&xin, 0, sizeof(xin));
    xin.x = view(x); xin.ix = ix; xin.Di = Di; xin.ones = ones; xin.N = N; xin.eff = eff; xin.active = active; xin.max_active = max_active;
    static_assert(sizeof(NgInput) <= sizeof(tdnnf_net::EarlyIn::xin), "EarlyIn::xin too small");
    if (n->early_on && n->early[comp].done == n->fb_count) {
      TDNNF_REQUIRE(memcmp(n->early[comp].xin, &xin, sizeof(xin)) == 0, "net_forward_backward: the input of component %s moved between minibatches",
                    n->comps[comp].name.c_str());
      if (n->early_group) {
        TDNNF_HIP(hipStreamWaitEvent(sw, n->ev_early, 0));
        CK(ng_stats_main_finish(n->ng_in[comp], xin, S.H_in, wsw, n->ws_bytes, sw));
      }
    } else {
      CK(ng_stats_main(n->ng_in[comp], xin, S.H_in, S.part_in, wsw, n->ws_bytes, sw));
    }
    if (n->early_on) {
      memcpy(n->early[comp].xin, &xin, sizeof(xin));
      n->early[comp].recorded = n->fb_count;
    }
    NgInput yin;
    memset(&yin, 0, sizeof(yin));
    yin.x = view(dyv); yin.ix.row_stride = 1; yin.ix.num_offsets = 1; yin.Di = Do; yin.N = N;
    if (fused_comp == comp) {
      fused_comp = -1;
      CK(ng_external_end(n->ng_out[comp], yin, S.H_out, wsw, n->ws_bytes, sw));
    } else {
      CK(ng_stats_main(n->ng_out[comp], yin, S.H_out, S.part_out, wsw, n->ws_bytes, sw));
    }
    if (grouped) {
      n->ng_cur.push_back(comp);
      CK(handed_off());
      if (from_tapgrad && n->wg_on) TDNNF_HIP(hipStreamWaitEvent(s, n->ev_pg[(n->pg_count - 1) & 3], 0));
      return TDNNF_OK;
    }
    TDNNF_HIP(hipEventRecord(n->ev_ngc, sw));
    TDNNF_HIP(hipStreamWaitEvent(n->s3, n->ev_ngc, 0));
    {
      SplitKScratchOverride side_scratch(n->s3_scratch, n->s3_scratch_bytes);
      CK(ng_stats_side(n->ng_in[comp], S.H_in, S.part_in, n->ng_side_ws, n->ngset_ws_bytes, n->s3));
      CK(ng_stats_side(n->ng_out[comp], S.H_out, S.part_out, n->ng_side_ws, n->ngset_ws_bytes, n->s3));
      CK(ng_project(n->ng_in[comp], n->ng_out[comp], T, Do, Dx, ldT, n->ngTmp, n->s3));
    }
    hipLaunchKernelGGL(ng_commit_kernel, dim3(grid_for((long long)Do * Dx, 256)), dim3(256), 0, n->s3, T, ldT, Do, ldw, ng_scale_dev(n->ng_in[comp]),
                       ng_scale_dev(n->ng_out[comp]), Wg(n, comp), bias_acc);
    CK(handed_off());
    if (from_tapgrad && n->wg_on) TDNNF_HIP(hipStreamWaitEvent(s, n->ev_pg[(n->pg_count - 1) & 3], 0));
    return TDNNF_OK;
  };
  ng_close = [&](int key) -> int {
    if (n->ng_cur.empty()) return TDNNF_OK;
    bool closes = false;
    for (auto &gb : n->buckets) closes = closes || gb.close_key == key;
    if (!closes) return TDNNF_OK;
    tdnnf_net::NgBucket *nb = nullptr;
    for (auto &b : n->ng_buckets)
      if (b.key == key) nb = &b;
    if (!nb) {
      std::vector<NgGroupComp> gc;
      for (int comp : n->ng_cur) {
        const CompDesc &cd = n->comps[comp];
        auto &S = n->ngc[comp];
        NgGroupComp g;
        g.in = n->ng_in[comp]; g.out = n->ng_out[comp];
        g.T = S.T; g.Do = cd.rows; g.ldw = cd.cols; g.Dx = cd.cols + (cd.has_bias ? 1 : 0); g.ldT = (g.Dx + 3) & ~3;
        g.bsum = cd.has_bias ? S.bsum : nullptr;
        g.H_in = S.H_in; g.H_out = S.H_out; g.part_in = S.part_in; g.part_out = S.part_out; g.N = S.N;
        g.W_acc = Wg(n, comp); g.bias_acc = Bg(n, comp);
        gc.push_back(g);
      }
      NgGroup *grp = nullptr;
      CK(ng_group_create(gc, &grp));
      n->ng_buckets.push_back(tdnnf_net::NgBucket{key, n->ng_cur, grp});
      nb = &n->ng_buckets.back();
    }
    TDNNF_REQUIRE(nb->comps == n->ng_cur, "net_forward_backward: the components of gradient bucket %d changed between minibatches", key);
    if (n->wg_on && n->pg_count > 0) {
      for (unsigned b = 1; b <= side_streams() && b <= n->pg_count; b++) TDNNF_HIP(hipStreamWaitEvent(n->s3, n->ev_pg[(n->pg_count - b) & 3], 0));
      if (caller_used) {
        TDNNF_HIP(hipEventRecord(n->ev_ngc, s));
        TDNNF_HIP(hipStreamWaitEvent(n->s3, n->ev_ngc, 0));
        caller_used = false;
      }
    } else {
      TDNNF_HIP(hipEventRecord(n->ev_ngc, s));
      TDNNF_HIP(hipStreamWaitEvent(n->s3, n->ev_ngc, 0));
    }
    if (n->early_any) TDNNF_HIP(hipStreamWaitEvent(n->s3, n->ev_early, 0));
    CK(ng_group_run(nb->group, n->s3));
    n->ng_cur.clear();
    return TDNNF_OK;
  };
  n->ng_cur.clear();
  tdnnf_mat d_pl = M(n->d_small, No, S);
  if (!early_at_fork) CK(finish_refreshes());
  const bool early_after_xent = !n->wg_on;
  if (!early_after_xent) CK(launch_early_in(2));
  for (int h = 1; h >= 0; h--) {
// ... 295 lines not shown
```

### tdnn-f_nas_amd/csrc/ng.h

```cpp
#pragma once
#include <hip/hip_runtime.h>

#include <vector>

#include "common.h"
#include "gemm_f32.h"
#include "tdnnf_hip.h"

struct tdnnf_ng {
  int rank, Rp, update_period, t, D, Dp, frozen;
  float num_samples_history, alpha, epsilon, delta, rho;
  std::vector<float> d;
  float *dev;
  float *W, *WT, *WWT, *wlast, *J, *W1, *Kd, *Ld, *Ad, *coeff, *tmpR, *neg_one, *scale_f;
  double *scal;
  float *pin;
  float *h_K, *h_L, *h_At, *h_coeff, *h_scale;
  double *h_tr0;
  float *scratch;
  size_t scratch_floats;
  int pending, job_done, job_N;
  hipEvent_t ev_job;
  hipEvent_t ev_wait;
  int device;
  bool cur_upd;
  int cur_N, cur_ones;
  std::vector<float> d_next;
  float rho_next;
  bool must_reorth;
  std::vector<double> sqrt_e1, inv_sqrt_e1;
};

namespace tdnnf {

struct NgInput {
  MatView x;
  tdnnf_tdnn_indexes ix;
  int Di, ones, N;
  const float *eff;
  const int *active;
  int max_active;
};

constexpr int kWtPadRows = 64;
struct NgRowdotArgs {
  const float *X;
  long long ldx;
  int row_stride;
  int nseg, Di;
  long long seg_off[16];
  const float *eff;
  const float *WT;
  int Rp;
  const float *bias;
  float *H;
  int ldh, N;
  double *part;
  int part_cap;
};
bool ng_rowdot_ok(const NgRowdotArgs &a);
hipError_t ng_rowdot(const NgRowdotArgs &a, hipStream_t s);

size_t ng_stats_workspace_bytes(int rank, int D, int K, int N);
int ng_stats_step(tdnnf_ng *ng, const NgInput &in, float *H, void *ws, size_t ws_bytes, hipStream_t s);
int ng_stats_main(tdnnf_ng *ng, const NgInput &in, float *H, double *part, void *ws, size_t ws_bytes, hipStream_t s);
int ng_stats_side(tdnnf_ng *ng, const float *H, const double *part, void *ws, size_t ws_bytes, hipStream_t s);
int ng_stats_main_prepare(tdnnf_ng *ng, const NgInput &in, float *H, double *part, hipStream_t s, RowsGemmArgs *out);
int ng_stats_main_finish(tdnnf_ng *ng, const NgInput &in, const float *H, void *ws, size_t ws_bytes, hipStream_t s);
int ng_finalize_if_ready(tdnnf_ng *ng, hipStream_t s, int *did);
int ng_external_begin(tdnnf_ng *ng, int D, const float **W, int *Rp, int *ldw, hipStream_t s);
int ng_external_end(tdnnf_ng *ng, const NgInput &in, const float *H, void *ws, size_t ws_bytes, hipStream_t s);
int ng_h_ld(const tdnnf_ng *ng);
int ng_dim(const tdnnf_ng *ng);
const float *ng_scale_dev(const tdnnf_ng *ng);
const float *ng_w_dev(const tdnnf_ng *ng);
int ng_w_ld(const tdnnf_ng *ng);

size_t ng_project_tmp_floats(const tdnnf_ng *in, const tdnnf_ng *out, int Do, int ldT);
int ng_project(tdnnf_ng *in, tdnnf_ng *out, float *T, int Do, int Dx, int ldT, float *tmp, hipStream_t s);


struct NgGroupComp {
  tdnnf_ng *in, *out;
  float *T;
  int Do, Dx, ldT, ldw;
  const float *bsum;
  const float *H_in, *H_out;
  const double *part_in, *part_out;
  int N;
  float *W_acc, *bias_acc;
};
struct NgGroup;
int ng_group_create(const std::vector<NgGroupComp> &comps, NgGroup **out);
void ng_group_destroy(NgGroup *g);
int ng_group_run(NgGroup *g, hipStream_t s);
struct NgFin;
int ng_fin_create(const std::vector<tdnnf_ng *> &objs, NgFin **out);
void ng_fin_destroy(NgFin *f);
int ng_fin_run(NgFin *f, hipStream_t s, bool wait, int *did);
bool ng_updating(const tdnnf_ng *ng);
void ng_pool_push(tdnnf_ng *ng);
void ng_pool_wait(tdnnf_ng *ng);
bool ng_pool_done(tdnnf_ng *ng);
int ng_finalize_one(tdnnf_ng *ng, hipStream_t s);

}
```

### tdnn-f_nas_amd/csrc/ng.hip

```cpp
#include "ng.h"

#include <math.h>
#include <string.h>

#include <condition_variable>
#include <deque>
#include <mutex>
#include <thread>
#include <vector>

#include "gemm_f32.h"
#include "host_linalg.h"


namespace tdnnf {
namespace {

inline int pad4(int x) { return (x + 3) & ~3; }
inline size_t pad4z(size_t x) { return (x + 3) & ~(size_t)3; }

__global__ void add_diag_rows_kernel(float *J, const float *W, const float *coeff, int R, int D) {
  const long long total = (long long)R * D;
  for (long long e = blockIdx.x * 256LL + threadIdx.x; e < total; e += gridDim.x * 256LL) J[e] += coeff[e / D] * W[e];
}
__global__ void derive_kernel(const float *W, int Rp, int D, int Dp, float *WT, float *wlast) {
  const long long total = (long long)D * Rp;
  for (long long e = blockIdx.x * 256LL + threadIdx.x; e < total; e += gridDim.x * 256LL) {
    const int dd = (int)(e / Rp), r = (int)(e % Rp);
    const float v = W[(size_t)r * Dp + dd];
    WT[e] = v;
    if (dd == D - 1) wlast[r] = v;
  }
}
__global__ void stack_taps_kernel(const float *W, int Rp, int Dp, int Di, int K, float *WP) {
  const long long total = (long long)K * Rp * Di;
  for (long long e = blockIdx.x * 256LL + threadIdx.x; e < total; e += gridDim.x * 256LL) {
    const int k = (int)(e % Di), ir = (int)(e / Di), i = ir / Rp, r = ir % Rp;
    WP[e] = W[(size_t)r * Dp + (size_t)i * Di + k];
  }
}
struct PformTaps {
  int K, o[kMaxSeg];
};
__global__ __launch_bounds__(256) void pform_combine_kernel(const float *P, int ldp, PformTaps tp, int Rp, const float *bias, float *H, int N,
                                                            const double *psum, double *part, int part_cap) {
  const int m0 = blockIdx.x * 128, per = Rp / 4;
  for (int e = threadIdx.x; e < 128 * per; e += 256) {
    const int m = m0 + e / per, q = e % per;
    if (m >= N) break;
    float4 v = make_float4(0.f, 0.f, 0.f, 0.f);
    if (bias) v = *reinterpret_cast<const float4 *>(bias + 4 * q);
    for (int i = 0; i < tp.K; i++) {
      const float4 t = *reinterpret_cast<const float4 *>(P + (size_t)(m + tp.o[i]) * ldp + i * Rp + 4 * q);
      v.x += t.x; v.y += t.y; v.z += t.z; v.w += t.w;
    }
    *reinterpret_cast<float4 *>(H + (size_t)m * Rp + 4 * q) = v;
  }
  if (threadIdx.x == 0) {
    double sacc = 0;
    for (int i = 0; i < tp.K; i++) sacc += psum[blockIdx.x + tp.o[i] / 128];
    part[blockIdx.x] = sacc;
  }
  for (int i = gridDim.x + blockIdx.x * 256 + threadIdx.x; i < part_cap; i += gridDim.x * 256) part[i] = 0.0;
}
__global__ void scatter_col_kernel(const float *v, int R, float *J, int ld, int col) {
  const int r = blockIdx.x * blockDim.x + threadIdx.x;
  if (r < R) J[(size_t)r * ld + col] = v[r];
}
__global__ __launch_bounds__(256) void ng_scalars_kernel(const double *partial, int nb, double ones_term, const float *L, const float *WWT,
                                                         int Rp, double *scal, float *scale_f) {
  __shared__ double red[3][4];
  double a = 0, b = 0, c = 0;
  for (int i = threadIdx.x; i < nb; i += 256) a += partial[i];
  for (int i = threadIdx.x; i < Rp * Rp; i += 256) {
    const double l = L[i];
    c += l * (double)WWT[i];
    if (i / Rp == i % Rp) b += l;
  }
  for (int o = 32; o > 0; o >>= 1) {
    a += __shfl_xor(a, o, 64);
    b += __shfl_xor(b, o, 64);
    c += __shfl_xor(c, o, 64);
  }
  if ((threadIdx.x & 63) == 0) {
    red[0][threadIdx.x >> 6] = a;
    red[1][threadIdx.x >> 6] = b;
    red[2][threadIdx.x >> 6] = c;
// ... 251 lines not shown
  }
  std::vector<float> Th(fRR, 0.f);
  for (int i = 0; i < R; i++)
    for (int j = 0; j <= i; j++) Th[(size_t)i * Rp + j] = (float)(Ci[(size_t)i * R + j] * ng->sqrt_e1[i] * ng->inv_sqrt_e1[j]);
  TDNNF_HIP(hipMemcpyAsync(ng->Ad, Th.data(), sizeof(float) * fRR, hipMemcpyHostToDevice, s));
  TDNNF_HIP(hipStreamSynchronize(s));
  RowsGemmArgs t2;
  memset(&t2, 0, sizeof(t2));
  t2.A = ng->Ad; t2.lda = Rp; t2.B = ng->W1; t2.ldb = Dp; t2.C = ng->J; t2.ldc = Dp; t2.M = Rp; t2.N = Dp; t2.init_mode = 2; t2.nseg = 1;
  t2.seg[0].klen = Rp; t2.seg[0].m_lo = 0; t2.seg[0].m_hi = Rp;
  TDNNF_HIP(rows_gemm(t2, false, s));
  TDNNF_HIP(hipMemcpyAsync(ng->W1, ng->J, sizeof(float) * fRD, hipMemcpyDeviceToDevice, s));
  return TDNNF_OK;
}

int finalize(tdnnf_ng *ng, hipStream_t s) {
  if (!ng->pending) return TDNNF_OK;
  pool().wait(ng);
  ng->pending = 0;
  const int Rp = ng->Rp, Dp = ng->Dp;
  const size_t fRR = (size_t)Rp * Rp, fRD = (size_t)Rp * Dp;
  TDNNF_HIP(hipMemcpyAsync(ng->coeff, ng->h_coeff, sizeof(float) * Rp, hipMemcpyHostToDevice, s));
  TDNNF_HIP(hipMemcpyAsync(ng->Ad, ng->h_At, sizeof(float) * fRR, hipMemcpyHostToDevice, s));
  hipLaunchKernelGGL(add_diag_rows_kernel, dim3(grid_for((long long)fRD, 256)), dim3(256), 0, s, ng->J, ng->W, ng->coeff, Rp, Dp);
  RowsGemmArgs w1;
  memset(&w1, 0, sizeof(w1));
  w1.A = ng->Ad; w1.lda = Rp; w1.B = ng->J; w1.ldb = Dp; w1.C = ng->W1; w1.ldc = Dp; w1.M = Rp; w1.N = Dp; w1.init_mode = 2; w1.nseg = 1;
  w1.seg[0].klen = Rp; w1.seg[0].m_lo = 0; w1.seg[0].m_hi = Rp;
  TDNNF_HIP(rows_gemm(w1, false, s));
  if (ng->must_reorth) {
    int rc = reorthogonalize(ng, s);
    if (rc) return rc;
  }
  TDNNF_HIP(hipMemcpyAsync(ng->W, ng->W1, sizeof(float) * fRD, hipMemcpyDeviceToDevice, s));
  ng->d = ng->d_next;
  ng->rho = ng->rho_next;
  return derive(ng, s);
}

constexpr int kPformSpanCap = 4096;
size_t pform_ws_bytes(int Rp, int Di, int K, int N) {
  if (K < 2 || K * Rp > 64) return 0;
  const size_t M = (size_t)N + kPformSpanCap;
  return sizeof(float) * ((size_t)K * Rp * Di + 64) + sizeof(float) * (M * K * Rp + 64) + sizeof(double) * ((size_t)rows_gemm_sumsq_blocks((int)M) + 8) + 256;
}
size_t stats_ws_bytes(int Rp, int Di, int K, int N) {
  const size_t part = ((size_t)rows_gemm_sumsq_blocks(N) * sizeof(double) + 63) & ~(size_t)63;
  return part + std::max(std::max(wgrad_workspace_bytes(Rp, Rp, 1, N), wgrad_workspace_bytes(Rp, Di, K, N)), pform_ws_bytes(Rp, Di, K, N));
}

int stats_after_h(tdnnf_ng *ng, const NgInput &in, const float *H, void *wg_ws, size_t wg_bytes, bool upd, hipStream_t s) {
  const int N = in.N, K = in.ix.num_offsets, Di = in.Di, Rp = ng->Rp, Dp = ng->Dp, D = ng->D;
  ng->cur_upd = upd;
  ng->cur_N = N;
  ng->cur_ones = in.ones;
  if (!upd) return TDNNF_OK;
  TDNNF_REQUIRE(wg_ws && wg_bytes >= wgrad_workspace_bytes(Rp, Di, K, N), "ng: workspace too small");
  TDNNF_HIP(hipMemsetAsync(ng->J, 0, sizeof(float) * (size_t)Rp * Dp, s));
  if (in.ones) TDNNF_HIP(hipMemsetAsync(ng->tmpR, 0, sizeof(float) * Rp, s));
  WgradArgs j;
  memset(&j, 0, sizeof(j));
  j.dY = H; j.lddy = Rp; j.X = in.x.data; j.ldx = in.x.stride; j.Do = Rp; j.Di = Di; j.K = K; j.N = N; j.row_stride = in.ix.row_stride;
  for (int i = 0; i < K; i++) j.row_offsets[i] = in.ix.row_offsets[i];
  j.coef = in.eff; j.scale = 1.f; j.G = ng->J; j.ldg = Dp; j.accumulate = 1; j.bias_acc = in.ones ? ng->tmpR : nullptr;
  j.active = in.active; j.max_active = in.max_active;
  TDNNF_HIP(wgrad(j, wg_ws, wg_bytes, s));
  if (in.ones) hipLaunchKernelGGL(scatter_col_kernel, dim3((Rp + 63) / 64), dim3(64), 0, s, ng->tmpR, Rp, ng->J, Dp, D - 1);
  return TDNNF_OK;
}

bool pform_ok(int Rp, const NgInput &in, size_t ws_bytes) {
  const int K = in.ix.num_offsets, N = in.N;
  if (!options().ng_pform || K < 2 || K * Rp > 64 || in.eff || in.active || in.ix.row_stride != 1 || N % 128 != 0 || N < 32768) return false;
  int lo = in.ix.row_offsets[0], hi = lo;
  for (int i = 1; i < K; i++) {
    lo = std::min(lo, in.ix.row_offsets[i]);
    hi = std::max(hi, in.ix.row_offsets[i]);
  }
  for (int i = 0; i < K; i++)
    if ((in.ix.row_offsets[i] - lo) % 128 != 0) return false;
  if (hi - lo > kPformSpanCap || in.Di % 4 != 0 || (in.x.stride % 4) != 0 || in.Di < 1024) return false;
  return ws_bytes >= pform_ws_bytes(Rp, in.Di, K, N);
}
int pform_pass(const float *W, int Rp, int Dp, const float *bias, const NgInput &in, float *H, double *part, void *ws, hipStream_t s) {
  const int K = in.ix.num_offsets, N = in.N, Di = in.Di;
  PformTaps tp;
  memset(&tp, 0, sizeof(tp));
  tp.K = K;
  int lo = in.ix.row_offsets[0], hi = lo;
  for (int i = 1; i < K; i++) {
    lo = std::min(lo, in.ix.row_offsets[i]);
    hi = std::max(hi, in.ix.row_offsets[i]);
  }
  for (int i = 0; i < K; i++) tp.o[i] = in.ix.row_offsets[i] - lo;
  const int M = N + (hi - lo);
  float *WP = (float *)ws;
  float *P = WP + (((size_t)K * Rp * Di + 63) & ~(size_t)63);
  double *psum = (double *)(P + (((size_t)M * K * Rp + 63) & ~(size_t)63));
  hipLaunchKernelGGL(stack_taps_kernel, dim3(grid_for((long long)K * Rp * Di, 256)), dim3(256), 0, s, W, Rp, Dp, Di, K, WP);
  RowsGemmArgs a;
  memset(&a, 0, sizeof(a));
  a.A = in.x.data + (size_t)lo * in.x.stride; a.lda = in.x.stride; a.B = WP; a.ldb = Di; a.C = P; a.ldc = K * Rp; a.M = M; a.N = K * Rp;
  a.init_mode = 2; a.sumsq = psum; a.nseg = 1;
  a.seg[0].klen = Di; a.seg[0].m_lo = 0; a.seg[0].m_hi = M;
  TDNNF_HIP(rows_gemm(a, true, s));
  hipLaunchKernelGGL(pform_combine_kernel, dim3(N / 128), dim3(256), 0, s, P, K * Rp, tp, Rp, bias, H, N, psum, part,
                     rows_gemm_sumsq_blocks(N));
  TDNNF_HIP(hipGetLastError());
  return TDNNF_OK;
}

RowsGemmArgs stats_h_args(const tdnnf_ng *ng, const NgInput &in, float *H, double *part) {
  const int N = in.N, K = in.ix.num_offsets, Di = in.Di, Rp = ng->Rp, Dp = ng->Dp;
  RowsGemmArgs a;
  memset(&a, 0, sizeof(a));
  a.A = in.x.data; a.lda = (long long)in.x.stride * in.ix.row_stride; a.B = ng->W; a.ldb = Dp; a.C = H; a.ldc = Rp; a.M = N; a.N = Rp;
  a.bias = in.ones ? ng->wlast : nullptr;
  a.init_mode = in.ones ? 1 : 2;
  a.coef = in.eff;
  a.sumsq = part;
  a.nseg = K;
  for (int i = 0; i < K; i++) {
    a.seg[i].a_off = (long long)in.ix.row_offsets[i] * in.x.stride;
    a.seg[i].b_off = (long long)i * Di;
    a.seg[i].klen = Di;
    a.seg[i].m_lo = 0;
    a.seg[i].m_hi = N;
  }
  return a;
}
int stats_main(tdnnf_ng *ng, const NgInput &in, float *H, double *part, void *wg_ws, size_t wg_bytes, bool upd, hipStream_t s) {
  const int N = in.N, K = in.ix.num_offsets, Di = in.Di, Rp = ng->Rp, Dp = ng->Dp;
  const RowsGemmArgs a = stats_h_args(ng, in, H, part);
  NgRowdotArgs v;
  memset(&v, 0, sizeof(v));
  v.X = in.x.data; v.ldx = in.x.stride; v.row_stride = in.ix.row_stride; v.nseg = K; v.Di = Di; v.eff = in.eff; v.WT = ng->WT; v.Rp = Rp;
  v.bias = in.ones ? ng->wlast : nullptr; v.H = H; v.ldh = Rp; v.N = N; v.part = part; v.part_cap = rows_gemm_sumsq_blocks(N);
  for (int i = 0; i < K; i++) v.seg_off[i] = (long long)in.ix.row_offsets[i] * in.x.stride;
  const int skip = options().ng_diag_skip;
  if (skip && ng->D != 0 && (((skip & 1) && K == 2 && Di >= 1024) || ((skip & 2) && !(K == 2 && Di >= 1024)))) {
    TDNNF_HIP(hipMemsetAsync(H, 0, sizeof(float) * (size_t)N * Rp, s));
    TDNNF_HIP(hipMemsetAsync(part, 0, sizeof(double) * rows_gemm_sumsq_blocks(N), s));
  } else if (pform_ok(Rp, in, wg_bytes)) {
    int rc = pform_pass(ng->W, Rp, Dp, in.ones ? ng->wlast : nullptr, in, H, part, wg_ws, s);
    if (rc) return rc;
  } else if (options().ng_valu && !in.active && ng_rowdot_ok(v)) {
    TDNNF_HIP(ng_rowdot(v, s));
  } else {
    TDNNF_HIP(rows_gemm(a, true, s));
  }
  return stats_after_h(ng, in, H, wg_ws, wg_bytes, upd, s);
}

int stats_side(tdnnf_ng *ng, const float *H, const double *part, void *wg_ws, size_t wg_bytes, hipStream_t s) {
  const int N = ng->cur_N, Rp = ng->Rp, Dp = ng->Dp;
  TDNNF_REQUIRE(wg_ws && wg_bytes >= wgrad_workspace_bytes(Rp, Rp, 1, N), "ng: workspace too small");
  WgradArgs w;
  memset(&w, 0, sizeof(w));
  w.dY = H; w.lddy = Rp; w.X = H; w.ldx = Rp; w.Do = Rp; w.Di = Rp; w.K = 1; w.N = N; w.row_stride = 1; w.scale = 1.f;
  w.G = ng->Ld; w.ldg = Rp; w.accumulate = 0;
  TDNNF_HIP(wgrad(w, wg_ws, wg_bytes, s));
  hipLaunchKernelGGL(ng_scalars_kernel, dim3(1), dim3(256), 0, s, part, rows_gemm_sumsq_blocks(N), ng->cur_ones ? (double)N : 0.0, ng->Ld, ng->WWT,
                     Rp, ng->scal, ng->scale_f);
  if (!ng->cur_upd) return TDNNF_OK;
  RowsGemmArgs k;
  memset(&k, 0, sizeof(k));
  k.A = ng->J; k.lda = Dp; k.B = ng->J; k.ldb = Dp; k.C = ng->Kd; k.ldc = Rp; k.M = Rp; k.N = Rp; k.init_mode = 2; k.nseg = 1;
  k.seg[0].klen = Dp; k.seg[0].m_lo = 0; k.seg[0].m_hi = Rp;
  TDNNF_HIP(rows_gemm(k, true, s));
  const size_t fRR = (size_t)Rp * Rp;
  TDNNF_HIP(hipMemcpyAsync(ng->h_K, ng->Kd, sizeof(float) * fRR, hipMemcpyDeviceToHost, s));
  TDNNF_HIP(hipMemcpyAsync(ng->h_L, ng->Ld, sizeof(float) * fRR, hipMemcpyDeviceToHost, s));
  TDNNF_HIP(hipMemcpyAsync(ng->h_tr0, ng->scal, sizeof(double), hipMemcpyDeviceToHost, s));
  ng->job_N = N;
  ng->job_done = 0;
  ng->pending = 1;
  TDNNF_HIP(hipEventRecord(ng->ev_job, s));
  ng->ev_wait = ng->ev_job;
  pool().push(ng);
  return TDNNF_OK;
}

int stats_core(tdnnf_ng *ng, const NgInput &in, float *H, void *ws, size_t ws_bytes, bool upd, hipStream_t s) {
  TDNNF_REQUIRE(ws && ws_bytes >= stats_ws_bytes(ng->Rp, in.Di, in.ix.num_offsets, in.N), "ng: workspace too small");
  double *part = (double *)ws;
  const size_t part_bytes = ((size_t)rows_gemm_sumsq_blocks(in.N) * sizeof(double) + 63) & ~(size_t)63;
  void *wg_ws = (char *)ws + part_bytes;
  const size_t wg_bytes = ws_bytes - part_bytes;
  int rc = stats_main(ng, in, H, part, wg_ws, wg_bytes, upd, s);
  if (rc) return rc;
  return stats_side(ng, H, part, wg_ws, wg_bytes, s);
}

int init_from(tdnnf_ng *ng, const NgInput &in, int D, float *H, void *ws, size_t ws_bytes, hipStream_t s) {
  int rc = init_default(ng, D, s);
  if (rc) return rc;
  if (ng->rank > 0) {
    const int iters = in.N <= ng->rank ? 1 : 3;
    for (int i = 0; i < iters; i++) {
      if ((rc = stats_core(ng, in, H, ws, ws_bytes, true, s))) return rc;
      if ((rc = finalize(ng, s))) return rc;
    }
  }
  ng->t = 0;
  return TDNNF_OK;
}

}

size_t ng_stats_workspace_bytes(int rank, int D, int K, int N) {
  const int Rp = pad4(std::max(1, std::min(rank, D - 1)));
  const int Di = K > 0 ? D / K : D;
  return stats_ws_bytes(Rp, Di, std::max(K, 1), N) + 64;
}
bool ng_updating(const tdnnf_ng *ng) { return updating(ng); }
void ng_pool_push(tdnnf_ng *ng) { pool().push(ng); }
void ng_pool_wait(tdnnf_ng *ng) { pool().wait(ng); }
bool ng_pool_done(tdnnf_ng *ng) { return pool().done(ng); }
int ng_finalize_one(tdnnf_ng *ng, hipStream_t s) {
  ProfClassOverride prof_as_ng(3);
  GemmPrecisionScope exact_f32(2);
  return finalize(ng, s);
}
int ng_h_ld(const tdnnf_ng *ng) { return ng->Rp; }
int ng_dim(const tdnnf_ng *ng) { return ng->D; }
const float *ng_scale_dev(const tdnnf_ng *ng) { return ng->scale_f; }
const float *ng_w_dev(const tdnnf_ng *ng) { return ng->W; }
int ng_w_ld(const tdnnf_ng *ng) { return ng->Dp; }

int ng_stats_step(tdnnf_ng *ng, const NgInput &in, float *H, void *ws, size_t ws_bytes, hipStream_t s) {
  const int K = in.ix.num_offsets, D = K * in.Di + (in.ones ? 1 : 0);
  TDNNF_REQUIRE(ng && H && in.N > 0 && K >= 1 && K <= kMaxSeg && in.Di > 0, "ng_stats_step: bad arguments");
  ProfClassOverride prof_as_ng(3);
  GemmPrecisionScope exact_f32(2);
  if (ng->D == 0) {
    int rc0 = init_from(ng, in, D, H, ws, ws_bytes, s);
    if (rc0) return rc0;
  }
  TDNNF_REQUIRE(ng->D == D, "ng: dimension changed from %d to %d", ng->D, D);
  if (ng->rank == 0) return TDNNF_OK;
  int rc = finalize(ng, s);
  if (rc) return rc;
  rc = stats_core(ng, in, H, ws, ws_bytes, updating(ng), s);
  ng->t += 1;
  return rc;
}

int ng_stats_main(tdnnf_ng *ng, const NgInput &in, float *H, double *part, void *ws, size_t ws_bytes, hipStream_t s) {
  const int K = in.ix.num_offsets, D = K * in.Di + (in.ones ? 1 : 0);
  TDNNF_REQUIRE(ng && H && part && in.N > 0 && K >= 1 && K <= kMaxSeg && in.Di > 0, "ng_stats_main: bad arguments");
  ProfClassOverride prof_as_ng(3);
  GemmPrecisionScope exact_f32(2);
  if (ng->D == 0) {
    int rc0 = init_from(ng, in, D, H, ws, ws_bytes, s);
    if (rc0) return rc0;
  }
  TDNNF_REQUIRE(ng->D == D, "ng: dimension changed from %d to %d", ng->D, D);
  ng->cur_N = 0;
  if (ng->rank == 0) return TDNNF_OK;
  int rc = finalize(ng, s);
  if (rc) return rc;
  return stats_main(ng, in, H, part, ws, ws_bytes, updating(ng), s);
}

int ng_stats_main_prepare(tdnnf_ng *ng, const NgInput &in, float *H, double *part, hipStream_t s, RowsGemmArgs *out) {
  const int K = in.ix.num_offsets, D = K * in.Di + (in.ones ? 1 : 0);
  TDNNF_REQUIRE(ng && H && part && out && in.N > 0 && K >= 1 && K <= kMaxSeg && ng->D == D, "ng_stats_main_prepare: bad arguments");
  if (ng->rank == 0) {
    memset(out, 0, sizeof(*out));
    ng->cur_N = 0;
    return TDNNF_OK;
  }
  ProfClassOverride prof_as_ng(3);
  GemmPrecisionScope exact_f32(2);
  ng->cur_N = 0;
  int rc = finalize(ng, s);
  if (rc) return rc;
  *out = stats_h_args(ng, in, H, part);
  return TDNNF_OK;
}
int ng_stats_main_finish(tdnnf_ng *ng, const NgInput &in, const float *H, void *ws, size_t ws_bytes, hipStream_t s) {
  TDNNF_REQUIRE(ng && H && ng->D != 0 && ng->rank > 0 && in.N > 0, "ng_stats_main_finish: bad arguments");
  ProfClassOverride prof_as_ng(3);
  GemmPrecisionScope exact_f32(2);
  return stats_after_h(ng, in, H, ws, ws_bytes, updating(ng), s);
}

int ng_finalize_if_ready(tdnnf_ng *ng, hipStream_t s, int *did) {
  *did = 0;
  if (!ng || ng->rank == 0 || !ng->pending || !pool().done(ng)) return TDNNF_OK;
  ProfClassOverride prof_as_ng(3);
  GemmPrecisionScope exact_f32(2);
  *did = 1;
  return finalize(ng, s);
}

int ng_external_begin(tdnnf_ng *ng, int D, const float **W, int *Rp, int *ldw, hipStream_t s) {
  TDNNF_REQUIRE(ng && W && Rp && ldw, "ng_external_begin: bad arguments");
  *W = nullptr;
  if (ng->D == 0 || ng->rank == 0) return TDNNF_OK;
  TDNNF_REQUIRE(ng->D == D, "ng: dimension changed from %d to %d", ng->D, D);
  ng->cur_N = 0;
  int rc = finalize(ng, s);
  if (rc) return rc;
  *W = ng->W;
  *Rp = ng->Rp;
  *ldw = ng->Dp;
  return TDNNF_OK;
}

int ng_external_end(tdnnf_ng *ng, const NgInput &in, const float *H, void *ws, size_t ws_bytes, hipStream_t s) {
  TDNNF_REQUIRE(ng && H && ng->D != 0 && ng->rank > 0 && in.N > 0, "ng_external_end: bad arguments");
  ProfClassOverride prof_as_ng(3);
  GemmPrecisionScope exact_f32(2);
  return stats_after_h(ng, in, H, ws, ws_bytes, updating(ng), s);
}

int ng_stats_side(tdnnf_ng *ng, const float *H, const double *part, void *ws, size_t ws_bytes, hipStream_t s) {
  TDNNF_REQUIRE(ng && H && part, "ng_stats_side: bad arguments");
  if (ng->rank == 0 || ng->cur_N == 0) return TDNNF_OK;
  ProfClassOverride prof_as_ng(3);
  GemmPrecisionScope exact_f32(2);
  int rc = stats_side(ng, H, part, ws, ws_bytes, s);
  ng->t += 1;
  return rc;
}

size_t ng_project_tmp_floats(const tdnnf_ng *in, const tdnnf_ng *out, int Do, int ldT) {
  const size_t q = in ? (size_t)Do * in->Rp : 0, p = out ? (size_t)out->Rp * ldT : 0;
  return std::max(q, p) + 16;
}

int ng_project(tdnnf_ng *in, tdnnf_ng *out, float *T, int Do, int Dx, int ldT, float *tmp, hipStream_t s) {
  TDNNF_REQUIRE(T && tmp && ldT % 4 == 0 && ldT >= Dx, "ng_project: bad arguments");
  ProfClassOverride prof_as_ng(3);
  GemmPrecisionScope exact_f32(2);
  if (in && in->rank > 0) {
    TDNNF_REQUIRE(in->D == Dx && in->Dp == ldT, "ng_project: input-side dimension mismatch");
    const int Rp = in->Rp;
    RowsGemmArgs q;
    memset(&q, 0, sizeof(q));
    q.A = T; q.lda = ldT; q.B = in->W; q.ldb = in->Dp; q.C = tmp; q.ldc = Rp; q.M = Do; q.N = Rp; q.init_mode = 2; q.nseg = 1;
    q.seg[0].klen = ldT; q.seg[0].m_lo = 0; q.seg[0].m_hi = Do;
    TDNNF_HIP(rows_gemm(q, true, s));
    RowsGemmArgs c;
    memset(&c, 0, sizeof(c));
    c.A = tmp; c.lda = Rp; c.B = in->W; c.ldb = in->Dp; c.C = T; c.ldc = ldT; c.M = Do; c.N = ldT; c.init_mode = 0; c.nseg = 1;
    c.coef = in->neg_one;
    c.seg[0].klen = Rp; c.seg[0].m_lo = 0; c.seg[0].m_hi = Do;
    TDNNF_HIP(rows_gemm(c, false, s));
  }
  if (out && out->rank > 0) {
    TDNNF_REQUIRE(out->D == Do, "ng_project: output-side dimension mismatch");
    const int Rp = out->Rp;
    RowsGemmArgs p;
    memset(&p, 0, sizeof(p));
    p.A = out->W; p.lda = out->Dp; p.B = T; p.ldb = ldT; p.C = tmp; p.ldc = ldT; p.M = Rp; p.N = ldT; p.init_mode = 2; p.nseg = 1;
    p.seg[0].klen = Do; p.seg[0].m_lo = 0; p.seg[0].m_hi = Rp;
    TDNNF_HIP(rows_gemm(p, false, s));
    RowsGemmArgs c;
    memset(&c, 0, sizeof(c));
    c.A = out->WT; c.lda = Rp; c.B = tmp; c.ldb = ldT; c.C = T; c.ldc = ldT; c.M = Do; c.N = ldT; c.init_mode = 0; c.nseg = 1;
    c.coef = out->neg_one;
    c.seg[0].klen = Rp; c.seg[0].m_lo = 0; c.seg[0].m_hi = Do;
    TDNNF_HIP(rows_gemm(c, false, s));
  }
  return TDNNF_OK;
}

}

using namespace tdnnf;

extern "C" {

const float *tdnnf_ng_scale_dev(const tdnnf_ng *ng) { return ng && ng->dev ? ng->scale_f : nullptr; }

size_t tdnnf_ng_stats_pass_workspace_bytes(int rank, int Di, int num_taps, int N) { return pform_ws_bytes((rank + 3) & ~3, Di, num_taps, N) + 64; }

int tdnnf_ng_stats_pass(const tdnnf_tdnn_indexes *ix, const tdnnf_mat *X, int Di, const float *eff, const float *WT, const float *W, int ldw,
                        const float *bias, tdnnf_mat *H, double *sumsq, int sumsq_cap, int use_valu, void *workspace, size_t workspace_bytes,
                        tdnnf_stream stream) {
  TDNNF_REQUIRE(ix && X && X->data && H && H->data && Di > 0 && ix->num_offsets >= 1 && ix->num_offsets <= kMaxSeg && ix->row_stride >= 1,
                "ng_stats_pass: bad arguments");
  const int K = ix->num_offsets, N = H->rows, Rp = H->cols;
  for (int i = 0; i < K; i++)
    TDNNF_REQUIRE(ix->row_offsets[i] >= 0 && (long long)(N - 1) * ix->row_stride + ix->row_offsets[i] < X->rows && Di <= X->cols,
                  "ng_stats_pass: tap %d reads outside X (%d x %d)", i, X->rows, X->cols);
  TDNNF_REQUIRE(!sumsq || sumsq_cap >= rows_gemm_sumsq_blocks(N), "ng_stats_pass: sumsq needs %d entries", rows_gemm_sumsq_blocks(N));
  hipStream_t s = (hipStream_t)stream;
  if (use_valu == 2) {
    NgInput in;
    memset(&in, 0, sizeof(in));
    in.x = view(X); in.ix = *ix; in.Di = Di; in.ones = bias ? 1 : 0; in.N = N; in.eff = eff;
    TDNNF_REQUIRE(W && ldw >= K * Di && sumsq && H->stride == Rp && workspace && pform_ok(Rp, in, workspace_bytes),
                  "ng_stats_pass: the one-pass form takes >= 2 taps of one matrix whole 128-row tiles apart, N %% 128 == 0, N >= 32768, taps x rank <= 64, no coefficients");
    return pform_pass(W, Rp, ldw, bias, in, H->data, sumsq, workspace, s);
  }
  if (use_valu) {
    NgRowdotArgs v;
    memset(&v, 0, sizeof(v));
    v.X = X->data; v.ldx = X->stride; v.row_stride = ix->row_stride; v.nseg = K; v.Di = Di; v.eff = eff; v.WT = WT; v.Rp = Rp;
    v.bias = bias; v.H = H->data; v.ldh = H->stride; v.N = N; v.part = sumsq; v.part_cap = sumsq_cap;
    for (int i = 0; i < K; i++) v.seg_off[i] = (long long)ix->row_offsets[i] * X->stride;
    TDNNF_REQUIRE(WT && ng_rowdot_ok(v), "ng_stats_pass: the vector-ALU kernel takes rank 20 / 40 / 80 and 16-byte aligned rows");
    TDNNF_HIP(ng_rowdot(v, s));
    return TDNNF_OK;
  }
  TDNNF_REQUIRE(W && ldw >= K * Di, "ng_stats_pass: the MFMA form needs W (rank x ldw)");
  GemmPrecisionScope exact_f32(2);
  RowsGemmArgs a;
  memset(&a, 0, sizeof(a));
  a.A = X->data; a.lda = (long long)X->stride * ix->row_stride; a.B = W; a.ldb = ldw; a.C = H->data; a.ldc = H->stride; a.M = N; a.N = Rp;
  a.bias = bias; a.init_mode = bias ? 1 : 2; a.coef = eff; a.sumsq = sumsq; a.nseg = K;
  for (int i = 0; i < K; i++) {
    a.seg[i].a_off = (long long)ix->row_offsets[i] * X->stride;
    a.seg[i].b_off = (long long)i * Di;
    a.seg[i].klen = Di;
    a.seg[i].m_lo = 0;
    a.seg[i].m_hi = N;
  }
  TDNNF_HIP(rows_gemm(a, true, s));
  return TDNNF_OK;
}

int tdnnf_ng_create(int rank, int update_period, float num_samples_history, float alpha, tdnnf_ng **out) {
  TDNNF_REQUIRE(out && rank >= 0 && update_period >= 1 && num_samples_history > 0 && alpha >= 0, "ng_create: bad configuration");
  tdnnf_ng *ng = new tdnnf_ng();
  ng->rank = rank;
  ng->Rp = 0;
  ng->update_period = update_period;
  ng->t = 0;
  ng->D = ng->Dp = 0;
  ng->frozen = 0;
  ng->num_samples_history = num_samples_history;
  ng->alpha = alpha;
  ng->epsilon = 1.0e-10f;
  ng->delta = 5.0e-04f;
  ng->rho = 0;
  ng->dev = nullptr;
  ng->pin = nullptr;
  ng->scratch = nullptr;
  ng->scratch_floats = 0;
  ng->pending = 0;
  ng->job_done = 0;
  ng->ev_job = nullptr;
  ng->ev_wait = nullptr;
  ng->must_reorth = false;
  *out = ng;
  return TDNNF_OK;
}

int tdnnf_ng_freeze(tdnnf_ng *ng, int freeze) {
  TDNNF_REQUIRE(ng, "ng_freeze: null object");
  ng->frozen = freeze ? 1 : 0;
  return TDNNF_OK;
}

void tdnnf_ng_destroy(tdnnf_ng *ng) {
  if (!ng) return;
  if (ng->pending) pool().wait(ng);
// ... 58 lines not shown
```

Measured before the change: 1.634 million.

## Fuse batchnorm-apply with natural-gradient input projection GEMM in one kernel

Adds a kernel that applies batchnorm/bypass to produce the layer output and, in the same pass, multiplies those rows by the stacked preconditioner tap weights on matrix cores, also accumulating per-tile sums of squares. The forward path routes eligible components through this fused sink so the later NG stats step only runs the combine stage. This avoids rereading the activation from memory for the separate product GEMM. In exchange it adds workspace, extra eligibility checks, an event wait, and a hand-written GEMM that may be slower than the tuned rows_gemm.

New measurement: 1.646 million (median of 6 runs). No clear change (+0.7%).

```diff
diff --git a/include/tdnnf_hip.h b/include/tdnnf_hip.h
--- a/include/tdnnf_hip.h
+++ b/include/tdnnf_hip.h
@@ -173,6 +173,10 @@
 int tdnnf_ng_stats_pass(const tdnnf_tdnn_indexes *ix, const tdnnf_mat *X, int Di, const float *eff_dev, const float *WT_dev,
                         const float *W_dev, int ldw, const float *bias_dev, tdnnf_mat *H, double *sumsq_dev, int sumsq_cap, int form,
                         void *workspace_dev, size_t workspace_bytes, tdnnf_stream);
+int tdnnf_bn_apply_in_ng(const tdnnf_mat *x, const float *memo_dev, int B, const float *mask_dev, const tdnnf_mat *prev, float bypass,
+                         tdnnf_mat *out, const tdnnf_tdnn_indexes *ix, const float *W_dev, int rank_padded, int ldw, int fused,
+                         float *P_dev, double *psum_dev, int *took, void *workspace_dev, size_t workspace_bytes, tdnnf_stream);
+void tdnnf_ng_in_fuse_counts(long long *fused, long long *separate);
 const float *tdnnf_ng_scale_dev(const tdnnf_ng *);
 
 size_t tdnnf_constrain_orthonormal_workspace_bytes(int rows, int cols);
diff --git a/tdnn-f_nas_amd/csrc/abi_tdnn.hip b/tdnn-f_nas_amd/csrc/abi_tdnn.hip
--- a/tdnn-f_nas_amd/csrc/abi_tdnn.hip
+++ b/tdnn-f_nas_amd/csrc/abi_tdnn.hip
@@ -80,7 +80,7 @@
   Options &o = options();
   if (!name) return nullptr;
   const struct { const char *n; int *p; } table[] = {{"ng_grouped", &o.ng_grouped}, {"ng_fuse", &o.ng_fuse}, {"ng_early_in", &o.ng_early_in},
-                                                     {"wgrad_stream", &o.wgrad_stream}, {"gemm_ring", &o.gemm_ring}, {"planes", &o.planes}, {"den_split", &o.den_split}, {"phase_events", &o.phase_events}, {"wgrad_lag", &o.wgrad_lag}, {"ng_bk", &o.ng_bk}, {"ng_valu", &o.ng_valu}, {"ng_pform", &o.ng_pform}, {"planes_group", &o.planes_group}, {"xent_behind_den", &o.xent_behind_den}, {"ng_early_fork", &o.ng_early_fork}, {"ng_diag_skip", &o.ng_diag_skip}, {"wgrad_small", &o.wgrad_small}, {"splitk_per_cu", &o.splitk_per_cu}, {"gemm_alt_taps", &o.gemm_alt_taps}, {"reverse_passes", &o.reverse_passes}, {"splitk_partial_round", &o.splitk_partial_round}, {"wgrad_on_caller", &o.wgrad_on_caller}, {"den_mw_test_abort", &o.den_mw_test_abort}, {"planes_check_bound", &o.planes_check_bound}, {"den_gamma_pairs", &o.den_gamma_pairs}};
+                                                     {"wgrad_stream", &o.wgrad_stream}, {"gemm_ring", &o.gemm_ring}, {"planes", &o.planes}, {"den_split", &o.den_split}, {"phase_events", &o.phase_events}, {"wgrad_lag", &o.wgrad_lag}, {"ng_bk", &o.ng_bk}, {"ng_valu", &o.ng_valu}, {"ng_pform", &o.ng_pform}, {"planes_group", &o.planes_group}, {"xent_behind_den", &o.xent_behind_den}, {"ng_early_fork", &o.ng_early_fork}, {"ng_diag_skip", &o.ng_diag_skip}, {"wgrad_small", &o.wgrad_small}, {"splitk_per_cu", &o.splitk_per_cu}, {"gemm_alt_taps", &o.gemm_alt_taps}, {"reverse_passes", &o.reverse_passes}, {"splitk_partial_round", &o.splitk_partial_round}, {"wgrad_on_caller", &o.wgrad_on_caller}, {"den_mw_test_abort", &o.den_mw_test_abort}, {"planes_check_bound", &o.planes_check_bound}, {"den_gamma_pairs", &o.den_gamma_pairs}, {"ng_in_fuse", &o.ng_in_fuse}};
   for (auto &e : table)
     if (strcmp(e.n, name) == 0) return e.p;
   return nullptr;
diff --git a/tdnn-f_nas_amd/csrc/common.h b/tdnn-f_nas_amd/csrc/common.h
--- a/tdnn-f_nas_amd/csrc/common.h
+++ b/tdnn-f_nas_amd/csrc/common.h
@@ -67,6 +67,7 @@
   int phase_events = 0;
   int den_split = -1;
   int den_gamma_pairs = 0;
+  int ng_in_fuse = 1;
 };
 Options &options();
 
diff --git a/tdnn-f_nas_amd/csrc/fused.h b/tdnn-f_nas_amd/csrc/fused.h
--- a/tdnn-f_nas_amd/csrc/fused.h
+++ b/tdnn-f_nas_amd/csrc/fused.h
@@ -8,8 +8,19 @@
   long long R;
   const float *rec;
 };
+struct NgInFuse {
+  const float *WP;
+  int KRp, ldw;
+  float *P;
+  int ldp;
+  double *psum;
+  int psum_cap;
+};
+bool bn_apply_in_ng_ok(MatView x, MatView prev, MatView out, int D, int period, const float *memo, const float *mask, const NgInFuse &g);
+bool bn_apply_in_ng_pays(int rows);
 hipError_t bn_apply_bypass(MatView x, const float *memo, int D, int period, MatView prev, float bypass, MatView out, hipStream_t s,
-                           const float *mask = nullptr, int B = 1, const PlanesSink *planes = nullptr);
+                           const float *mask = nullptr, int B = 1, const PlanesSink *planes = nullptr,
+                           const NgInFuse *ng_in = nullptr);
 
 struct BwdPlanes {
   void *P;
diff --git a/tdnn-f_nas_amd/csrc/fused.hip b/tdnn-f_nas_amd/csrc/fused.hip
--- a/tdnn-f_nas_amd/csrc/fused.hip
+++ b/tdnn-f_nas_amd/csrc/fused.hip
@@ -72,6 +72,146 @@
   }
 }
 
+template <bool MASK>
+__global__ __launch_bounds__(256, 2) void bn_apply_in_ng_kernel(MatView x, const float *mean, const float *scale, int D, MatView prev, float bypass,
+                                                                MatView out, const float *mask, int B, NgInFuse g, int rev) {
+  typedef float acc_t __attribute__((ext_vector_type(16)));
+  constexpr int BM = 128, BN = 64, BK = 32, LDT = BK + 4, A_TILE = BM * LDT, B_TILE = BN * LDT;
+  __shared__ __attribute__((aligned(16))) float smem[2 * (A_TILE + B_TILE)];
+  float *As = smem, *Bs = smem + 2 * A_TILE;
+  const int tile = rev ? (int)gridDim.x - 1 - (int)blockIdx.x : (int)blockIdx.x;
+  const int m0 = tile * BM;
+  const int t = threadIdx.x, lane = t & 63, wave = t >> 6, li = lane & 31, lh = lane >> 5;
+  const int r0 = t >> 3, c4 = (t & 7) * 4;
+  acc_t acc[2];
+#pragma unroll
+  for (int j = 0; j < 2; j++)
+#pragma unroll
+    for (int r = 0; r < 16; r++) acc[j][r] = 0.f;
+
+  const float *xp[4], *pp[4], *mp[4], *bp[2];
+  float *op[4];
+  bool rv[4], bv[2];
+#pragma unroll
+  for (int j = 0; j < 4; j++) {
+    const int m = m0 + r0 + 32 * j;
+    rv[j] = m < x.rows;
+    const long long mm = rv[j] ? m : 0;
+    xp[j] = x.data + mm * x.stride + c4;
+    pp[j] = prev.data ? prev.data + mm * prev.stride + c4 : nullptr;
+    op[j] = out.data + mm * out.stride + c4;
+    mp[j] = MASK ? mask + (long long)(mm % B) * D + c4 : nullptr;
+  }
+#pragma unroll
+  for (int j = 0; j < 2; j++) {
+    const int nn = r0 + 32 * j;
+    bv[j] = nn < g.KRp;
+    bp[j] = g.WP + (long long)(bv[j] ? nn : 0) * g.ldw + c4;
+  }
+  const float4 zero4 = make_float4(0.f, 0.f, 0.f, 0.f);
+  const bool has_prev = prev.data != nullptr;
+  float4 xv[4], pv[4] = {zero4, zero4, zero4, zero4}, mv[4], rb[2], mu, sc;
+  float ssq = 0.f;
+  auto load_tile = [&](int kc) {
+#pragma unroll
+    for (int j = 0; j < 4; j++) {
+      xv[j] = *reinterpret_cast<const float4 *>(xp[j] + kc);
+      if (has_prev) pv[j] = *reinterpret_cast<const float4 *>(pp[j] + kc);
+      if (MASK) mv[j] = *reinterpret_cast<const float4 *>(mp[j] + kc);
+    }
+    mu = *reinterpret_cast<const float4 *>(mean + kc + c4);
+    sc = *reinterpret_cast<const float4 *>(scale + kc + c4);
+#pragma unroll
+    for (int j = 0; j < 2; j++) rb[j] = *reinterpret_cast<const float4 *>(bp[j] + kc);
+  };
+  auto store_tile = [&](int buf, int kc) {
+    float4 ra[4];
+    {
+#pragma clang fp contract(off)
+#pragma unroll
+      for (int j = 0; j < 4; j++) {
+        const float k0 = MASK ? mv[j].x : 1.f, k1 = MASK ? mv[j].y : 1.f, k2 = MASK ? mv[j].z : 1.f, k3 = MASK ? mv[j].w : 1.f;
+        ra[j].x = __builtin_fmaf(bypass, pv[j].x, ((xv[j].x - mu.x) * sc.x) * k0);
+        ra[j].y = __builtin_fmaf(bypass, pv[j].y, ((xv[j].y - mu.y) * sc.y) * k1);
+        ra[j].z = __builtin_fmaf(bypass, pv[j].z, ((xv[j].z - mu.z) * sc.z) * k2);
+        ra[j].w = __builtin_fmaf(bypass, pv[j].w, ((xv[j].w - mu.w) * sc.w) * k3);
+        if (rv[j]) {
+          *reinterpret_cast<float4 *>(op[j] + kc) = ra[j];
+        } else {
+          ra[j].x = 0.f; ra[j].y = 0.f; ra[j].z = 0.f; ra[j].w = 0.f;
+        }
+      }
+      float q0 = 0.f, q1 = 0.f;
+#pragma unroll
+      for (int j = 0; j < 4; j++) {
+        asm volatile("v_fmac_f32 %0, %2, %2\n v_fmac_f32 %1, %3, %3\n v_fmac_f32 %0, %4, %4\n v_fmac_f32 %1, %5, %5"
+                     : "+v"(q0), "+v"(q1)
+                     : "v"(ra[j].x), "v"(ra[j].y), "v"(ra[j].z), "v"(ra[j].w));
+      }
+      ssq += q0 + q1;
+    }
+    float *as = As + buf * A_TILE, *bs = Bs + buf * B_TILE;
+#pragma unroll
+    for (int j = 0; j < 4; j++) *reinterpret_cast<float4 *>(as + (r0 + 32 * j) * LDT + c4) = ra[j];
+#pragma unroll
+    for (int j = 0; j < 2; j++)
+      *reinterpret_cast<float4 *>(bs + (r0 + 32 * j) * LDT + c4) = make_float4(bv[j] ? rb[j].x : 0.f, bv[j] ? rb[j].y : 0.f, bv[j] ? rb[j].z : 0.f, bv[j] ? rb[j].w : 0.f);
+  };
+  auto compute = [&](int buf) {
+    const float *as = As + buf * A_TILE + (wave * 32 + li) * LDT + lh * 4;
+    const float *bs = Bs + buf * B_TILE + li * LDT + lh * 4;
+#pragma unroll
+    for (int kg = 0; kg < BK / 8; kg++) {
+      const float4 a = *reinterpret_cast<const float4 *>(as + kg * 8);
+      float4 b[2];
+#pragma unroll
+      for (int j = 0; j < 2; j++) b[j] = *reinterpret_cast<const float4 *>(bs + j * 32 * LDT + kg * 8);
+#pragma unroll
+      for (int j = 0; j < 2; j++) {
+        acc[j] = __builtin_amdgcn_mfma_f32_32x32x2f32(a.x, b[j].x, acc[j], 0, 0, 0);
+        acc[j] = __builtin_amdgcn_mfma_f32_32x32x2f32(a.y, b[j].y, acc[j], 0, 0, 0);
+        acc[j] = __builtin_amdgcn_mfma_f32_32x32x2f32(a.z, b[j].z, acc[j], 0, 0, 0);
+        acc[j] = __builtin_amdgcn_mfma_f32_32x32x2f32(a.w, b[j].w, acc[j], 0, 0, 0);
+      }
+    }
+  };
+
+  load_tile(0);
+  store_tile(0, 0);
+  __syncthreads();
+  int buf = 0;
+  for (int kc = BK;; kc += BK) {
+    const bool more = kc < D;
+    if (more) load_tile(kc);
+    compute(buf);
+    if (!more) break;
+    store_tile(buf ^ 1, kc);
+    __syncthreads();
+    buf ^= 1;
+  }
+  __syncthreads();
+  {
+    double v = ssq;
+    for (int o = 32; o > 0; o >>= 1) v += __shfl_xor(v, o, 64);
+    double *red = reinterpret_cast<double *>(smem);
+    if (lane == 0) red[wave] = v;
+    __syncthreads();
+    if (t == 0) g.psum[tile] = (red[0] + red[1]) + (red[2] + red[3]);
+    if (tile == 0)
+      for (int i = (int)gridDim.x + t; i < g.psum_cap; i += 256) g.psum[i] = 0.0;
+  }
+#pragma unroll
+  for (int j = 0; j < 2; j++) {
+    const int col = j * 32 + li;
+    if (col >= g.KRp) continue;
+#pragma unroll
+    for (int r = 0; r < 16; r++) {
+      const int m = m0 + wave * 32 + (r & 3) + 8 * (r >> 2) + 4 * lh;
+      if (m < x.rows) g.P[(long long)m * g.ldp + col] = acc[j][r];
+    }
+  }
+}
+
 template <int VEC, bool RELU_STATS>
 __global__ __launch_bounds__(256) void bn_relu_bwd_reduce_kernel(MatView x, MatView dz, const float *mean, const float *scale,
                                                                  int rows_per_chunk, int chunks, float *partial, const float *mask, int B) {
@@ -424,9 +564,26 @@
 
 }
 
+bool bn_apply_in_ng_ok(MatView x, MatView prev, MatView out, int D, int period, const float *memo, const float *mask, const NgInFuse &g) {
+  const auto al16 = [](const void *p) { return (reinterpret_cast<uintptr_t>(p) & 15) == 0; };
+  return x.rows >= 1 && x.cols == D && out.cols == D && out.rows == x.rows && period >= D && D % 32 == 0 && vec4_ok(x) && vec4_ok(out) &&
+         (!prev.data || (vec4_ok(prev) && prev.rows == x.rows && prev.cols == D)) && memo && al16(memo) && (!mask || al16(mask)) && g.WP && al16(g.WP) &&
+         g.ldw % 4 == 0 && g.ldw >= D && g.KRp >= 1 && g.KRp <= 64 && g.P && g.ldp >= g.KRp && g.psum && g.psum_cap >= (x.rows + 127) / 128;
+}
+bool bn_apply_in_ng_pays(int rows) { return bn_relu_bwd_ng_pays(rows); }
+
 hipError_t bn_apply_bypass(MatView x, const float *memo, int D, int period, MatView prev, float bypass, MatView out, hipStream_t s, const float *mask, int B,
-                           const PlanesSink *planes) {
+                           const PlanesSink *planes, const NgInFuse *ng_in) {
   if (x.rows == 0) return hipSuccess;
+  if (ng_in) {
+    if (planes || !bn_apply_in_ng_ok(x, prev, out, D, period, memo, mask, *ng_in)) return hipErrorInvalidValue;
+    ProfHbmRange prof(4, 4.0 * x.rows * (x.cols * (prev.data ? 3.0 : 2.0) + ng_in->KRp), s);
+    const dim3 grid((x.rows + 127) / 128);
+    const int rev = options().reverse_passes & 1;
+    if (mask) hipLaunchKernelGGL((bn_apply_in_ng_kernel<true>), grid, dim3(256), 0, s, x, memo, memo + 2 * D, D, prev, bypass, out, mask, B, *ng_in, rev);
+    else hipLaunchKernelGGL((bn_apply_in_ng_kernel<false>), grid, dim3(256), 0, s, x, memo, memo + 2 * D, D, prev, bypass, out, mask, B, *ng_in, rev);
+    return hipGetLastError();
+  }
   const bool vec = vec4_ok(x) && vec4_ok(out) && (!prev.data || vec4_ok(prev)) && D % 4 == 0 && (reinterpret_cast<uintptr_t>(memo) & 15) == 0 &&
                    (!mask || (reinterpret_cast<uintptr_t>(mask) & 15) == 0);
   const long long work = (long long)x.rows * (vec ? x.cols / 4 : x.cols);
diff --git a/tdnn-f_nas_amd/csrc/net.h b/tdnn-f_nas_amd/csrc/net.h
--- a/tdnn-f_nas_amd/csrc/net.h
+++ b/tdnn-f_nas_amd/csrc/net.h
@@ -111,6 +111,8 @@
     float *H_in = nullptr, *H_out = nullptr, *T = nullptr, *bsum = nullptr;
     double *part_in = nullptr, *part_out = nullptr;
     int N = 0;
+    void *pf_ws = nullptr;
+    size_t pf_bytes = 0;
   };
   std::vector<NgComp> ngc;
   float *ng_bsum_all = nullptr;
@@ -118,6 +120,7 @@
   float *ngTmp = nullptr;
   void *ng_side_ws = nullptr;
   size_t ngset_ws_bytes = 0;
+  size_t ng_in_fuse_bytes = 0;
   struct NgBucket {
     int key;
     std::vector<int> comps;
@@ -149,6 +152,7 @@
   struct EarlyIn {
     unsigned char xin[256];
     long long recorded = -1, done = -1;
+    long long fused = -1;
   };
   std::vector<EarlyIn> early;
   long long fb_count = 0;
diff --git a/tdnn-f_nas_amd/csrc/net.hip b/tdnn-f_nas_amd/csrc/net.hip
--- a/tdnn-f_nas_amd/csrc/net.hip
+++ b/tdnn-f_nas_amd/csrc/net.hip
@@ -422,6 +422,7 @@
   n->orthoT = tall ? A.take<float>(tall + 16) : nullptr;
   size_t ng_ws = 0;
   n->ngc.assign(n->comps.size(), tdnnf_net::NgComp());
+  n->ng_in_fuse_bytes = 0;
   if (n->cfg.use_natural_gradient) {
     size_t mtmp = 0;
     auto comp_ng = [&](int comp, int K, int rows) {
@@ -440,6 +441,11 @@
       S.bsum = nullptr;
       S.part_in = A.take<double>((size_t)rows_gemm_sumsq_blocks(rows) + 8);
       S.part_out = A.take<double>((size_t)rows_gemm_sumsq_blocks(rows) + 8);
+      if (options().ng_in_fuse && K >= 2 && !cd.has_bias && rows >= 32768 && rows % 128 == 0 && cd.cols % K == 0 && cd.cols / K >= 1024) {
+        S.pf_bytes = ng_in_fuse_workspace_bytes(rank_in, cd.cols / K, K, rows);
+        S.pf_ws = S.pf_bytes ? A.take<char>(S.pf_bytes + 64) : nullptr;
+        n->ng_in_fuse_bytes += S.pf_bytes;
+      }
     };
     const int No_ = n->Tout * B;
     comp_ng(n->tdnn1.comp, 1, N0);
@@ -1318,13 +1324,41 @@
     po->P = ps.P; po->R = R; po->lead = lead; po->kb_alloc = kb_alloc; po->scale = ps.scale;
     return TDNNF_OK;
   };
+  bool in_fuse_waited = false;
+  auto in_fuse_sink = [&](int consumer, const MatView &x, const float *memo, const MatView &byp, const tdnnf_mat &out, const float *mask, NgInFuse *sink) -> bool {
+    if (!options().ng_in_fuse || !c.use_natural_gradient || !n->early_on || n->early_group || consumer < 0 || pl_on) return false;
+    auto &E = n->early[consumer];
+    auto &S = n->ngc[consumer];
+    if (!S.pf_ws || !S.H_in || E.recorded != n->fb_count - 1 || E.done == n->fb_count || !n->ng_in[consumer] || !n->ng_out[consumer] ||
+        ng_dim(n->ng_in[consumer]) == 0 || ng_dim(n->ng_out[consumer]) == 0 || n->comps[consumer].lr_factor == 0.f)
+      return false;
+    if (!bn_apply_in_ng_pays(out.rows)) return false;
+    NgInput xin;
+    memcpy(&xin, E.xin, sizeof(xin));
+    if (early_refresh && !in_fuse_waited) {
+      if (hipStreamWaitEvent(s, n->ev_fin, 0) != hipSuccess) return false;
+      in_fuse_waited = true;
+    }
+    NgInFuse g;
+    memset(&g, 0, sizeof(g));
+    {
+      g.WP = reinterpret_cast<const float *>(S.pf_ws); g.KRp = xin.ix.num_offsets * ng_h_ld(n->ng_in[consumer]); g.ldw = xin.Di;
+      g.P = reinterpret_cast<float *>(S.pf_ws); g.ldp = g.KRp; g.psum = reinterpret_cast<double *>(S.pf_ws); g.psum_cap = rows_gemm_sumsq_blocks(out.rows);
+      if (!bn_apply_in_ng_ok(x, byp, view(&out), Hd, ldpad(Hd), memo, mask, g)) return false;
+    }
+    if (!ng_in_fuse_begin(n->ng_in[consumer], xin, view(&out), S.pf_ws, S.pf_bytes, s, sink)) return false;
+    E.fused = n->fb_count;
+    return true;
+  };
   auto bn_apply_planes = [&](const tdnnf_mat &x, const float *memo, const MatView &byp, float bypass, const tdnnf_mat &out, const float *mask, const FroBound &fb,
-                             PlanesOperand *po) -> int {
+                             PlanesOperand *po, int consumer = -1) -> int {
     *po = PlanesOperand();
     auto it = (pl_on && np == 2 && fb.blocks > 0 && (fb.add_coef == 0.f || fb.add_rec) && out.cols == Hd && out.stride == ldpad(Hd)) ? n->plane_slots.find(out.data)
                                                                                                                                          : n->plane_slots.end();
     if (it == n->plane_slots.end()) {
-      TDNNF_HIP(bn_apply_bypass(view(&x), memo, Hd, ldpad(Hd), byp, bypass, view(&out), s, mask, B));
+      NgInFuse sink;
+      const bool fuse = in_fuse_sink(consumer, view(&x), memo, byp, out, mask, &sink);
+      TDNNF_HIP(bn_apply_bypass(view(&x), memo, Hd, ldpad(Hd), byp, bypass, view(&out), s, mask, B, nullptr, fuse ? &sink : nullptr));
       return TDNNF_OK;
     }
     tdnnf_net::PlaneSlot &ps = it->second;
@@ -1390,7 +1424,7 @@
   }
   fb_next.mul = mask_max;
   PlanesOperand po_next;
-  CK(bn_apply_planes(t1r, n->t1_bn_memo, none, 0.f, t1b, mask_of(0), fb_next, &po_next));
+  CK(bn_apply_planes(t1r, n->t1_bn_memo, none, 0.f, t1b, mask_of(0), fb_next, &po_next, n->layers.empty() ? -1 : n->layers[0].lin.comp));
   float *prev = n->t1_bn;
   int layer_no = 0;
   for (auto &L : n->layers) {
@@ -1457,7 +1491,9 @@
       x = tdnnf_mat{L.relu_out, L.gout.n, byp.cols, B * ldpad(Hd)};
       out = tdnnf_mat{L.noop_out, L.gout.n, byp.cols, B * ldpad(Hd)};
     }
-    if (byp.rows == relu.rows) CK(bn_apply_planes(x, L.bn_memo, view(&byp), c.bypass_scale, out, mask_of(layer_no), fb_next, &po_next));
+    if (byp.rows == relu.rows)
+      CK(bn_apply_planes(x, L.bn_memo, view(&byp), c.bypass_scale, out, mask_of(layer_no), fb_next, &po_next,
+                         layer_no < (int)n->layers.size() ? n->layers[layer_no].lin.comp : -1));
     else TDNNF_HIP(bn_apply_bypass(view(&x), L.bn_memo, Hd, ldpad(Hd), view(&byp), c.bypass_scale, view(&out), s, mask_of(layer_no), B));
     prev = L.noop_out;
   }
@@ -1533,7 +1569,8 @@
       }
       NgInput xin;
       memcpy(&xin, E.xin, sizeof(xin));
-      CK(ng_stats_main(n->ng_in[comp], xin, n->ngc[comp].H_in, n->ngc[comp].part_in, n->ws4, n->ws_bytes, n->s4));
+      CK(ng_stats_main(n->ng_in[comp], xin, n->ngc[comp].H_in, n->ngc[comp].part_in, n->ws4, n->ws_bytes, n->s4,
+                       E.fused == n->fb_count ? n->ngc[comp].pf_ws : nullptr));
       E.done = n->fb_count;
     }
     if (forked) {
@@ -1757,7 +1794,8 @@
         CK(ng_stats_main_finish(n->ng_in[comp], xin, S.H_in, wsw, n->ws_bytes, sw));
       }
     } else {
-      CK(ng_stats_main(n->ng_in[comp], xin, S.H_in, S.part_in, wsw, n->ws_bytes, sw));
+      const bool fused_in = n->early_on && n->early[comp].fused == n->fb_count && memcmp(n->early[comp].xin, &xin, sizeof(xin)) == 0;
+      CK(ng_stats_main(n->ng_in[comp], xin, S.H_in, S.part_in, wsw, n->ws_bytes, sw, fused_in ? S.pf_ws : nullptr));
     }
     if (n->early_on) {
       memcpy(n->early[comp].xin, &xin, sizeof(xin));
diff --git a/tdnn-f_nas_amd/csrc/ng.h b/tdnn-f_nas_amd/csrc/ng.h
--- a/tdnn-f_nas_amd/csrc/ng.h
+++ b/tdnn-f_nas_amd/csrc/ng.h
@@ -4,6 +4,7 @@
 #include <vector>
 
 #include "common.h"
+#include "fused.h"
 #include "gemm_f32.h"
 #include "tdnnf_hip.h"
 
@@ -63,7 +64,10 @@
 
 size_t ng_stats_workspace_bytes(int rank, int D, int K, int N);
 int ng_stats_step(tdnnf_ng *ng, const NgInput &in, float *H, void *ws, size_t ws_bytes, hipStream_t s);
-int ng_stats_main(tdnnf_ng *ng, const NgInput &in, float *H, double *part, void *ws, size_t ws_bytes, hipStream_t s);
+int ng_stats_main(tdnnf_ng *ng, const NgInput &in, float *H, double *part, void *ws, size_t ws_bytes, hipStream_t s, void *pform_done = nullptr);
+size_t ng_in_fuse_workspace_bytes(int rank, int Di, int K, int N);
+bool ng_in_fuse_begin(tdnnf_ng *ng, const NgInput &in, MatView out, void *pws, size_t pws_bytes, hipStream_t s, NgInFuse *sink);
+void ng_in_fuse_counts(long long *fused, long long *separate);
 int ng_stats_side(tdnnf_ng *ng, const float *H, const double *part, void *ws, size_t ws_bytes, hipStream_t s);
 int ng_stats_main_prepare(tdnnf_ng *ng, const NgInput &in, float *H, double *part, hipStream_t s, RowsGemmArgs *out);
 int ng_stats_main_finish(tdnnf_ng *ng, const NgInput &in, const float *H, void *ws, size_t ws_bytes, hipStream_t s);
diff --git a/tdnn-f_nas_amd/csrc/ng.hip b/tdnn-f_nas_amd/csrc/ng.hip
--- a/tdnn-f_nas_amd/csrc/ng.hip
+++ b/tdnn-f_nas_amd/csrc/ng.hip
@@ -3,6 +3,7 @@
 #include <math.h>
 #include <string.h>
 
+#include <atomic>
 #include <condition_variable>
 #include <deque>
 #include <mutex>
@@ -420,30 +421,50 @@
   if (hi - lo > kPformSpanCap || in.Di % 4 != 0 || (in.x.stride % 4) != 0 || in.Di < 1024) return false;
   return ws_bytes >= pform_ws_bytes(Rp, in.Di, K, N);
 }
-int pform_pass(const float *W, int Rp, int Dp, const float *bias, const NgInput &in, float *H, double *part, void *ws, hipStream_t s) {
+enum { kPformPrepare = 1, kPformProduct = 2, kPformCombine = 4, kPformAll = 7 };
+struct PformPlan {
+  PformTaps tp;
+  int lo, M;
+  float *WP, *P;
+  double *psum;
+};
+PformPlan pform_plan(int Rp, const NgInput &in, void *ws, int p_rows = 0) {
   const int K = in.ix.num_offsets, N = in.N, Di = in.Di;
-  PformTaps tp;
-  memset(&tp, 0, sizeof(tp));
-  tp.K = K;
+  PformPlan pl;
+  memset(&pl, 0, sizeof(pl));
+  pl.tp.K = K;
   int lo = in.ix.row_offsets[0], hi = lo;
   for (int i = 1; i < K; i++) {
     lo = std::min(lo, in.ix.row_offsets[i]);
     hi = std::max(hi, in.ix.row_offsets[i]);
   }
-  for (int i = 0; i < K; i++) tp.o[i] = in.ix.row_offsets[i] - lo;
-  const int M = N + (hi - lo);
-  float *WP = (float *)ws;
-  float *P = WP + (((size_t)K * Rp * Di + 63) & ~(size_t)63);
-  double *psum = (double *)(P + (((size_t)M * K * Rp + 63) & ~(size_t)63));
-  hipLaunchKernelGGL(stack_taps_kernel, dim3(grid_for((long long)K * Rp * Di, 256)), dim3(256), 0, s, W, Rp, Dp, Di, K, WP);
-  RowsGemmArgs a;
-  memset(&a, 0, sizeof(a));
-  a.A = in.x.data + (size_t)lo * in.x.stride; a.lda = in.x.stride; a.B = WP; a.ldb = Di; a.C = P; a.ldc = K * Rp; a.M = M; a.N = K * Rp;
-  a.init_mode = 2; a.sumsq = psum; a.nseg = 1;
-  a.seg[0].klen = Di; a.seg[0].m_lo = 0; a.seg[0].m_hi = M;
-  TDNNF_HIP(rows_gemm(a, true, s));
-  hipLaunchKernelGGL(pform_combine_kernel, dim3(N / 128), dim3(256), 0, s, P, K * Rp, tp, Rp, bias, H, N, psum, part,
-                     rows_gemm_sumsq_blocks(N));
+  for (int i = 0; i < K; i++) pl.tp.o[i] = in.ix.row_offsets[i] - lo;
+  pl.lo = lo;
+  pl.M = N + (hi - lo);
+  pl.WP = (float *)ws;
+  pl.P = pl.WP + (((size_t)K * Rp * Di + 63) & ~(size_t)63);
+  pl.psum = (double *)(pl.P + (((size_t)std::max(pl.M, p_rows) * K * Rp + 63) & ~(size_t)63));
+  return pl;
+}
+std::atomic<long long> g_pform_separate{0}, g_pform_fused{0};
+int pform_pass(const float *W, int Rp, int Dp, const float *bias, const NgInput &in, float *H, double *part, void *ws, hipStream_t s, int steps = kPformAll,
+               int p_rows = 0) {
+  const int K = in.ix.num_offsets, N = in.N, Di = in.Di;
+  const PformPlan pl = pform_plan(Rp, in, ws, p_rows);
+  if (steps & kPformPrepare)
+    hipLaunchKernelGGL(stack_taps_kernel, dim3(grid_for((long long)K * Rp * Di, 256)), dim3(256), 0, s, W, Rp, Dp, Di, K, pl.WP);
+  if (steps & kPformProduct) {
+    RowsGemmArgs a;
+    memset(&a, 0, sizeof(a));
+    a.A = in.x.data + (long long)pl.lo * in.x.stride; a.lda = in.x.stride; a.B = pl.WP; a.ldb = Di; a.C = pl.P; a.ldc = K * Rp; a.M = pl.M; a.N = K * Rp;
+    a.init_mode = 2; a.sumsq = pl.psum; a.nseg = 1;
+    a.seg[0].klen = Di; a.seg[0].m_lo = 0; a.seg[0].m_hi = pl.M;
+    TDNNF_HIP(rows_gemm(a, true, s));
+    g_pform_separate++;
+  }
+  if (steps & kPformCombine)
+    hipLaunchKernelGGL(pform_combine_kernel, dim3(N / 128), dim3(256), 0, s, pl.P, K * Rp, pl.tp, Rp, bias, H, N, pl.psum, part,
+                       rows_gemm_sumsq_blocks(N));
   TDNNF_HIP(hipGetLastError());
   return TDNNF_OK;
 }
@@ -467,7 +488,7 @@
   }
   return a;
 }
-int stats_main(tdnnf_ng *ng, const NgInput &in, float *H, double *part, void *wg_ws, size_t wg_bytes, bool upd, hipStream_t s) {
+int stats_main(tdnnf_ng *ng, const NgInput &in, float *H, double *part, void *wg_ws, size_t wg_bytes, bool upd, hipStream_t s, void *pform_done = nullptr) {
   const int N = in.N, K = in.ix.num_offsets, Di = in.Di, Rp = ng->Rp, Dp = ng->Dp;
   const RowsGemmArgs a = stats_h_args(ng, in, H, part);
   NgRowdotArgs v;
@@ -476,7 +497,10 @@
   v.bias = in.ones ? ng->wlast : nullptr; v.H = H; v.ldh = Rp; v.N = N; v.part = part; v.part_cap = rows_gemm_sumsq_blocks(N);
   for (int i = 0; i < K; i++) v.seg_off[i] = (long long)in.ix.row_offsets[i] * in.x.stride;
   const int skip = options().ng_diag_skip;
-  if (skip && ng->D != 0 && (((skip & 1) && K == 2 && Di >= 1024) || ((skip & 2) && !(K == 2 && Di >= 1024)))) {
+  if (pform_done) {
+    int rc = pform_pass(ng->W, Rp, Dp, in.ones ? ng->wlast : nullptr, in, H, part, pform_done, s, kPformCombine);
+    if (rc) return rc;
+  } else if (skip && ng->D != 0 && (((skip & 1) && K == 2 && Di >= 1024) || ((skip & 2) && !(K == 2 && Di >= 1024)))) {
     TDNNF_HIP(hipMemsetAsync(H, 0, sizeof(float) * (size_t)N * Rp, s));
     TDNNF_HIP(hipMemsetAsync(part, 0, sizeof(double) * rows_gemm_sumsq_blocks(N), s));
   } else if (pform_ok(Rp, in, wg_bytes)) {
@@ -584,9 +608,27 @@
   return rc;
 }
 
-int ng_stats_main(tdnnf_ng *ng, const NgInput &in, float *H, double *part, void *ws, size_t ws_bytes, hipStream_t s) {
+size_t ng_in_fuse_workspace_bytes(int rank, int Di, int K, int N) { return pform_ws_bytes(pad4(rank), Di, K, N); }
+void ng_in_fuse_counts(long long *fused, long long *separate) {
+  if (fused) *fused = g_pform_fused.load();
+  if (separate) *separate = g_pform_separate.load();
+}
+bool ng_in_fuse_begin(tdnnf_ng *ng, const NgInput &in, MatView out, void *pws, size_t pws_bytes, hipStream_t s, NgInFuse *sink) {
+  const int K = in.ix.num_offsets;
+  if (!ng || !pws || ng->D == 0 || ng->rank == 0 || ng->pending || ng->D != K * in.Di + (in.ones ? 1 : 0) || !pform_ok(ng->Rp, in, pws_bytes)) return false;
+  const PformPlan pl = pform_plan(ng->Rp, in, pws);
+  if (in.x.data + (long long)pl.lo * in.x.stride != out.data || pl.M != out.rows || in.x.stride != out.stride || in.Di != out.cols) return false;
+  if (pform_pass(ng->W, ng->Rp, ng->Dp, nullptr, in, nullptr, nullptr, pws, s, kPformPrepare) != TDNNF_OK) return false;
+  sink->WP = pl.WP; sink->KRp = K * ng->Rp; sink->ldw = in.Di; sink->P = pl.P; sink->ldp = K * ng->Rp; sink->psum = pl.psum;
+  sink->psum_cap = rows_gemm_sumsq_blocks(pl.M);
+  g_pform_fused++;
+  return true;
+}
+
+int ng_stats_main(tdnnf_ng *ng, const NgInput &in, float *H, double *part, void *ws, size_t ws_bytes, hipStream_t s, void *pform_done) {
   const int K = in.ix.num_offsets, D = K * in.Di + (in.ones ? 1 : 0);
   TDNNF_REQUIRE(ng && H && part && in.N > 0 && K >= 1 && K <= kMaxSeg && in.Di > 0, "ng_stats_main: bad arguments");
+  TDNNF_REQUIRE(!pform_done || (ng->D != 0 && ng->rank > 0 && !ng->pending), "ng_stats_main: the preconditioner changed behind a fused input pass");
   ProfClassOverride prof_as_ng(3);
   GemmPrecisionScope exact_f32(2);
   if (ng->D == 0) {
@@ -598,7 +640,7 @@
   if (ng->rank == 0) return TDNNF_OK;
   int rc = finalize(ng, s);
   if (rc) return rc;
-  return stats_main(ng, in, H, part, ws, ws_bytes, updating(ng), s);
+  return stats_main(ng, in, H, part, ws, ws_bytes, updating(ng), s, pform_done);
 }
 
 int ng_stats_main_prepare(tdnnf_ng *ng, const NgInput &in, float *H, double *part, hipStream_t s, RowsGemmArgs *out) {
@@ -715,6 +757,55 @@
 const float *tdnnf_ng_scale_dev(const tdnnf_ng *ng) { return ng && ng->dev ? ng->scale_f : nullptr; }
 
 size_t tdnnf_ng_stats_pass_workspace_bytes(int rank, int Di, int num_taps, int N) { return pform_ws_bytes((rank + 3) & ~3, Di, num_taps, N) + 64; }
+
+void tdnnf_ng_in_fuse_counts(long long *fused, long long *separate) { ng_in_fuse_counts(fused, separate); }
+
+int tdnnf_bn_apply_in_ng(const tdnnf_mat *x, const float *memo, int B, const float *mask, const tdnnf_mat *prev, float bypass, tdnnf_mat *out,
+                         const tdnnf_tdnn_indexes *ix, const float *W, int Rp, int ldw, int fused, float *P_out, double *psum_out, int *took,
+                         void *workspace, size_t workspace_bytes, tdnnf_stream stream) {
+  TDNNF_REQUIRE(x && x->data && out && out->data && memo && ix && W && took && B >= 1 && x->rows == out->rows && x->cols == out->cols &&
+                    ix->num_offsets >= 1 && ix->num_offsets <= kMaxSeg && Rp >= 4 && Rp % 4 == 0 && ldw >= ix->num_offsets * x->cols,
+                "bn_apply_in_ng: bad arguments");
+  hipStream_t s = (hipStream_t)stream;
+  const int D = x->cols, K = ix->num_offsets;
+  int lo = ix->row_offsets[0], hi = lo;
+  for (int i = 1; i < K; i++) {
+    lo = std::min(lo, ix->row_offsets[i]);
+    hi = std::max(hi, ix->row_offsets[i]);
+  }
+  TDNNF_REQUIRE(lo >= 0 && hi - lo < out->rows, "bn_apply_in_ng: the taps leave no rows");
+  MatView pv;
+  memset(&pv, 0, sizeof(pv));
+  if (prev && prev->data) pv = view(prev);
+  NgInput in;
+  memset(&in, 0, sizeof(in));
+  in.x = view(out); in.ix = *ix; in.Di = D; in.N = (out->rows - hi) / 128 * 128;
+  const int ld = (D + 3) & ~3;
+  *took = -1;
+  if (lo != 0 || in.N <= 0 || !workspace || !pform_ok(Rp, in, workspace_bytes) || out->rows > in.N + kPformSpanCap) {
+    TDNNF_HIP(bn_apply_bypass(view(x), memo, D, ld, pv, bypass, view(out), s, mask, B));
+    return TDNNF_OK;
+  }
+  const PformPlan pl = pform_plan(Rp, in, workspace, out->rows);
+  NgInFuse g;
+  g.WP = pl.WP; g.KRp = K * Rp; g.ldw = D; g.P = pl.P; g.ldp = K * Rp; g.psum = pl.psum; g.psum_cap = rows_gemm_sumsq_blocks(pl.M);
+  int rc = pform_pass(W, Rp, ldw, nullptr, in, nullptr, nullptr, workspace, s, kPformPrepare, out->rows);
+  if (rc) return rc;
+  if (fused && pl.M <= out->rows && out->rows - pl.M < 128 && bn_apply_in_ng_ok(view(x), pv, view(out), D, ld, memo, mask, g) && bn_apply_in_ng_pays(out->rows)) {
+    TDNNF_HIP(bn_apply_bypass(view(x), memo, D, ld, pv, bypass, view(out), s, mask, B, nullptr, &g));
+    g_pform_fused++;
+    *took = 1;
+  } else {
+    TDNNF_HIP(bn_apply_bypass(view(x), memo, D, ld, pv, bypass, view(out), s, mask, B));
+    GemmPrecisionScope exact_f32(2);
+    rc = pform_pass(W, Rp, ldw, nullptr, in, nullptr, nullptr, workspace, s, kPformProduct, out->rows);
+    if (rc) return rc;
+    *took = 0;
+  }
+  if (P_out) TDNNF_HIP(hipMemcpyAsync(P_out, pl.P, sizeof(float) * (size_t)pl.M * K * Rp, hipMemcpyDeviceToDevice, s));
+  if (psum_out) TDNNF_HIP(hipMemcpyAsync(psum_out, pl.psum, sizeof(double) * ((pl.M + 127) / 128), hipMemcpyDeviceToDevice, s));
+  return TDNNF_OK;
+}
 
 int tdnnf_ng_stats_pass(const tdnnf_tdnn_indexes *ix, const tdnnf_mat *X, int Di, const float *eff, const float *WT, const float *W, int ldw,
                         const float *bias, tdnnf_mat *H, double *sumsq, int sumsq_cap, int use_valu, void *workspace, size_t workspace_bytes,
```
